# apple/ml-4m

Hardware: AMD Instinct MI355X
Metric: multimodal tokens/sec (4M-B train step, whole job) (higher is better)
Workload: dtype bf16; 1 GPU; 4M-B mod7 (fm_base_12e_12d_swiglu_nobias, 360.8M params, 8 input / 7 target modalities) masked-modeling train step, 224^2 token grids, 128 input + 128 target tokens/sample, AdamW; model=fm_base_12e_12d_swiglu_nobias, per_gpu_batch=256, global_batch=256, seq_len=256, parallelism=dp1

## Files before the change

include/fourm_hip.h:

```cpp
#ifndef FOURM_HIP_H
#define FOURM_HIP_H
#include <stdint.h>

#ifdef __cplusplus
extern "C" {
#endif

#define FM_ABI_VERSION 11
int fm_abi_version(void);
const char* fm_last_error(void);

enum fm_epilogue {
    FM_EPI_BF16 = 0,
    FM_EPI_GELU = 1,
    FM_EPI_RESIDUAL = 2,
    FM_EPI_SWIGLU = 3,
    FM_EPI_F32 = 4,
    FM_EPI_TANH = 5,
    FM_EPI_SWIGLU_BWD = 6,
    FM_EPI_GELU_BWD = 7,
    FM_EPI_QUICK_GELU = 8,
    FM_EPI_RELU = 9,
    FM_EPI_RELU_BWD = 10
};
// ... 97 lines not shown
    FM_KIND_SEQ = 2,
    FM_KIND_SEQ_EMB = 3
};
typedef struct fm_mod_desc {
    const void* ids;
    const void* mask;
    const void* dam;
    const void* table;
    const void* pos;
    const void* mod_emb;
    const void* proj_bias;
    int32_t L;
    int32_t kind, ids_are_i64, mod_id;
    int32_t max_len;
    int32_t shifted;
    int32_t mask_stride, id_stride;
    int32_t patch, channels, grid_w, orig_dim;
    int32_t head_index;
    int32_t pad_;
} fm_mod_desc;

typedef struct fm_select_desc {
    fm_mod_desc mods[FM_MAX_MODS];
    int32_t n_mods, batch, dim, n_keep, n_reg, total_len, is_decoder;
    int32_t raw;
    const void* reg_tokens;
    const void* mask_token;
    void* tokens;
    void* emb;
    void* x0;
    void* out_mask;
    void* out_mod;
    void* slot_mod;
    void* slot_src;
    void* slot_pos;
    void* target_ids;
    void* out_cs;
    void* out_mod_pre;
    void* out_mod_index;
    void* patch_rows;
    void* seqemb_rows;
    int32_t patch_ld, seqemb_ld;
    int32_t rows_f32;
    int32_t pad2_;
} fm_select_desc;
int fm_select_embed(const fm_select_desc* desc, void* stream);

typedef struct fm_embed_bwd_mod {
    void* d_table;
    void* d_pos;
    void* d_mod_emb;
    void* d_proj_bias;
    int32_t kind, has_padding_idx, padding_idx, pad_;
} fm_embed_bwd_mod;
typedef struct fm_embed_bwd_desc {
    fm_embed_bwd_mod mods[FM_MAX_MODS];
    const void* dx;
    const void* slot_mod; const void* slot_src; const void* slot_pos;
    void* d_mask_token;
    void* d_reg_tokens;
    int32_t n_mods, batch, dim, Nt, lddx, is_decoder;
} fm_embed_bwd_desc;
int fm_embed_bwd(const fm_embed_bwd_desc* desc, void* stream);

int fm_dense_decoder_mask(const int32_t* cs, const int16_t* mod, void* out, int B, int M, int causal, int use_cs,
                          int use_sep, void* stream);

enum fm_loss_type { FM_LOSS_MOD = 0, FM_LOSS_TOKEN = 1 };
#define FM_SEG_ROWS 256
int fm_segment_rows(const int32_t* head_of_row, int R, int n_heads, int32_t* seg_start, int32_t* seg_count,
                    int32_t* perm, int32_t* row_to_padded, int32_t* tile_group, int Rp, void* stream);
int fm_gather_rows(const void* src, int ld_src, const int32_t* perm, void* dst, int ld_dst, int Rp, int D, void* stream);
int fm_cross_entropy(void* logits, int ldl, const int32_t* perm, const int32_t* tile_group, const int64_t* target_ids,
                     const int32_t* vocab, const int32_t* seg_start, const int32_t* seg_count, const void* grad_scale,
                     int loss_type, int n_heads, int Rp, int max_vocab, void* row_loss, void* row_lse, void* head_loss,
                     void* total_loss, int write_grad, void* stream);

int fm_swiglu_bwd(const void* da, int ldda, const void* gu, int ldgu, void* dgu, int lddgu, int R, int H, int Hp, void* stream);
int fm_gelu_bwd(const void* dh, int lddh, const void* pre, int ldp, void* dpre, int lddp, int R, int H, int Hp, void* stream);
typedef struct fm_shadow_desc {
    const void* src; void* dst;
    int32_t ld_src, ld_dst, rows, cols, transpose, tile_start;
    const void* col_scale;
    int32_t dst_f32, reserved;
} fm_shadow_desc;
int fm_shadow_refresh(const fm_shadow_desc* descs, int n_descs, int total_tiles, void* stream);
#define FM_FOLD_MAX_JOBS 48
typedef struct fm_fold_grad_job {
    const void* dWp; const void* W; const void* gamma; void* gW; void* ggamma;
    int32_t rows, cols, ld_dwp, reserved;
} fm_fold_grad_job;
int fm_fold_colscale_grad(const fm_fold_grad_job* jobs, int n_jobs, void* stream);

int fm_cast_pad(const void* src, int ld_src, void* dst, int ld_dst, int rows, int cols, void* stream);
int fm_transpose_cast_pad(const void* src, int ld_src, void* dst, int ld_dst, int dst_cols, int rows, int cols, void* stream);
int fm_colsum(const void* dy, int ldy, void* db, int R, int N, void* stream);
int fm_f32_to_bf16(const void* src, void* dst, int64_t n, void* stream);
int fm_bf16_to_f32_scaled(const void* src, void* dst, int64_t n, float scale, void* stream);
int fm_add_bf16_f32(const void* x, const void* delta, void* out, int64_t n, void* stream);
int fm_scale_rows_bf16(void* x, int ld, const void* scale, int rows_per_sample, int R, int N, void* stream);

int fm_vit_patch_rows(const void* pixels, void* rows, int ld, int B, int C, int H, int W, int P, int rows_f32, void* stream);
int fm_vit_emb_rows(const void* pos, const void* mod_emb, void* x, int ldx, int B, int Np, int D, void* stream);
int fm_vit_colsum(const void* dy, int ldy, void* db, int R, int N, void* ws, int64_t ws_bytes, void* stream);

int fm_clip_embed_ln(const void* patches, int ldp, int patches_f32, const void* cls, const void* pos, const void* w, const void* b,
                     void* out, int ldo, int B, int G, int D, float eps, void* stream);

enum { FM_FEAT_COSINE = 0, FM_FEAT_L1 = 1 };
int fm_feat_distance(const void* pred, int ldp, const void* tgt, int ldt, int B, int T, int D, int mode, void* loss, void* dpred, int lddp,
                     void* stream);
int fm_quick_gelu_bwd(const void* da, int ldda, const void* pre, int ldp, void* dpre, int lddp, int R, int H, int Hp, void* stream);
int fm_quick_gelu_bwd_f32(const void* da, int ldda, const void* pre, int ldp, void* dpre, int lddp, int R, int H, void* stream);
int fm_clip_embed_ln_bwd(const void* dy, int lddy, const void* patches, int ldp, int patches_f32, const void* pos, const void* w,
                         void* d_patches, int lddp, int B, int G, int D, float eps, void* stream);
int fm_tap_add(void* g, int ldg, void* g_bf, int ldgb, const void* dtap, int ldt, const void* row_scale, int rows_per_sample, int R, int D,
               void* stream);

#define FM_LPIPS_CHUNK 64
int fm_lpips_stem(const void* img, const void* mul, const void* add, const void* w, const void* bias, void* out, int ldo, int is_f32, int B, int H,
                  int W, void* stream);
int fm_lpips_stem_bwd(const void* d, int ldd, int is_f32, const void* w, const void* mul, const void* row_scale, void* dimg, int B, int H, int W,
                      void* stream);
int fm_maxpool2x2_nhwc(const void* x, int ldx, void* y, int ldy, int is_f32, int B, int H, int W, int C, void* stream);
int fm_lpips_distance(const void* pred, int ldp, const void* tgt, int ldt, int is_f32, const void* w, int B, int P, int C, void* loss, void* dpred,
                      int lddp, void* scratch, void* stream);
int fm_lpips_tap_bwd(const void* act, int lda, const void* din, int ldi, const void* dtap, int ldt, const void* dpool, int ldp, void* d, int ldd,
                     int is_f32, int B, int H, int W, int C, void* stream);

int fm_lora_apply(const void* x, int ldx, const void* down, int64_t down_sr, int64_t down_sk, const void* up, int64_t up_sn, int64_t up_sr,
                  void* y, int ldy, float scale, void* p_out, int R, int K, int N, int r, int x_f32, int y_f32, void* stream);
int fm_lora_grad(const void* a, int lda, const void* b, void* out, int64_t out_sn, int64_t out_sr, float scale, int accumulate,
                 int R, int n, int r, int a_f32, void* stream);

int fm_adamw(void* p, const void* g, void* m, void* v, int64_t n, float lr, float beta1, float beta2, float eps,
             float weight_decay, int64_t step, const void* grad_mult, const void* hyper, void* sumsq, void* stream);
#define FM_ADAMW_CHUNK 8192
typedef struct fm_adamw_job {
    void* p; const void* g; void* m; void* v; void* dst_plain; void* dst_t;
    int32_t rows, cols, ld_plain, ld_t, tile_start, pad_;
} fm_adamw_job;
int fm_adamw_shadow(const fm_adamw_job* jobs, int n_jobs, int total_tiles, float lr, float beta1, float beta2, float eps,
                    float weight_decay, int64_t step, const void* grad_mult, const void* hyper, void* sumsq, void* stream);
int fm_sumsq(const void* x, int64_t n, void* out, void* stream);
int fm_clip_coef(const void* sumsq, float max_norm, void* norm_out, void* coef_out, void* stream);

int fm_sample_tokens(const void* logits, int ld, int logits_are_f32, int R, int V, float temperature, int top_k, float top_p,
                     const void* uniforms, void* out_ids, void* out_prob, void* stream);
int fm_guidance_combine(const void* uncond, int ldu, int uncond_is_f32, const void* cond, int ldc, int cond_is_f32, float weight,
                        void* out, int ldo, int R, int V, int accumulate, void* stream);
int fm_maskgit_commit(const void* prob, const void* samples, const int32_t* mod_pos, int B, int N, int num_select, void* tensor,
                      int tensor_is_i64, int L, void* input_mask, void* target_mask, int32_t* top_idx, void* stream);

typedef struct fm_gemm_f32_args {
    const void* X; const void* W; const void* W2; void* out; void* out2; const void* res; const void* bias; const void* bias2;
    int64_t sxm, sxk, swn, swk;
    int32_t M, N, K, ldo, ldo2, ldr, Hp, epilogue, accumulate, max_N, seg_rows, n_groups;
    const fm_gemm_group* groups; const int32_t* tile_group; const int32_t* seg_start; const int32_t* seg_count;
} fm_gemm_f32_args;
int fm_gemm_f32(const fm_gemm_f32_args* args, void* stream);
int fm_attn_f32_fwd(const fm_attn_args* args, void* stream);
int fm_attn_f32_bwd(const fm_attn_args* args, void* stream);
int fm_layernorm_bwd_f32(const void* dy, int lddy, const int32_t* dy_row_map, const void* x, int ldx, const void* w, const void* mean,
                         const void* rstd, const void* dres, void* dx, int lddx, void* dx2, int lddx2, void* dw, void* db, int R, int D,
                         void* stream);
int fm_headnorm_f32_fwd(const void* x, int ldx, const void* w, const void* b, void* y, int ldy, void* stats, int R, int H, float eps, void* stream);
int fm_headnorm_f32_bwd(const void* dy, int lddy, const void* x, int ldx, const void* w, const void* stats, void* dx, int lddx, void* dw, void* db,
// ... 198 lines not shown
```

ml-4m_amd/csrc/elementwise.hip:

```cpp
#include "common.h"
#include "fourm_hip.h"

namespace {

__device__ __forceinline__ float4 ld_bf4(const bf16_t* p) {
    const uint2 v = *(const uint2*)p;
    return make_float4(bf2f((bf16_t)(v.x & 0xffff)), bf2f((bf16_t)(v.x >> 16)), bf2f((bf16_t)(v.y & 0xffff)), bf2f((bf16_t)(v.y >> 16)));
}
__device__ __forceinline__ void st_bf4(bf16_t* p, float a, float b, float c, float d) {
    *(uint2*)p = make_uint2(pack2bf(a, b), pack2bf(c, d));
}
__device__ __forceinline__ float sigmoid_f(float x) { return 1.0f / (1.0f + __expf(-x)); }

__global__ __launch_bounds__(256) void swiglu_bwd_kernel(const bf16_t* __restrict__ da, int ldda, const bf16_t* __restrict__ gu, int ldgu,
                                                         bf16_t* __restrict__ dgu, int lddgu, int R, int H, int Hp, int nt) {
    const int cpr = Hp / 8;
    const size_t total = (size_t)R * cpr;
    for (size_t i = (size_t)blockIdx.x * 256 + threadIdx.x; i < total; i += (size_t)gridDim.x * 256) {
        const int r = i / cpr, c = (i % cpr) * 8;
        typedef __attribute__((ext_vector_type(4))) unsigned int u4_t;
        uint4 dp, gp, up;
        if (nt & 2) { const u4_t t = __builtin_nontemporal_load((const u4_t*)(da + (size_t)r * ldda + c)); dp = make_uint4(t[0], t[1], t[2], t[3]); }
        else dp = *(const uint4*)(da + (size_t)r * ldda + c);
        if (nt & 1) {
            const u4_t t = __builtin_nontemporal_load((const u4_t*)(gu + (size_t)r * ldgu + c)), v = __builtin_nontemporal_load((const u4_t*)(gu + (size_t)r * ldgu + Hp + c));
            gp = make_uint4(t[0], t[1], t[2], t[3]); up = make_uint4(v[0], v[1], v[2], v[3]);
        } else { gp = *(const uint4*)(gu + (size_t)r * ldgu + c); up = *(const uint4*)(gu + (size_t)r * ldgu + Hp + c); }
        const uint32_t dw[4] = {dp.x, dp.y, dp.z, dp.w}, gw[4] = {gp.x, gp.y, gp.z, gp.w}, uw[4] = {up.x, up.y, up.z, up.w};
        uint32_t og[4], ou[4];
#pragma unroll
        for (int q = 0; q < 4; ++q) {
            float dg[2], du[2];
#pragma unroll
            for (int e = 0; e < 2; ++e) {
                const float dv = bf2f((bf16_t)(e ? dw[q] >> 16 : dw[q] & 0xffff));
                const float gv = bf2f((bf16_t)(e ? gw[q] >> 16 : gw[q] & 0xffff));
                const float uv = bf2f((bf16_t)(e ? uw[q] >> 16 : uw[q] & 0xffff));
                const float sg = sigmoid_f(gv);
                const float sl = bfround(gv * sg);
                const float ds = bfround(dv * uv);
                const bool live = c + 2 * q + e < H;
                du[e] = live ? dv * sl : 0.f;
                dg[e] = live ? ds * (sg * (1.0f + gv * (1.0f - sg))) : 0.f;
            }
            og[q] = pack2bf(dg[0], dg[1]); ou[q] = pack2bf(du[0], du[1]);
        }
        *(uint4*)(dgu + (size_t)r * lddgu + c) = make_uint4(og[0], og[1], og[2], og[3]);
        *(uint4*)(dgu + (size_t)r * lddgu + Hp + c) = make_uint4(ou[0], ou[1], ou[2], ou[3]);
    }
}

__global__ __launch_bounds__(256) void gelu_bwd_kernel(const bf16_t* __restrict__ dh, int lddh, const bf16_t* __restrict__ pre, int ldp,
                                                       bf16_t* __restrict__ dpre, int lddp, int R, int H, int Hp) {
    const int cpr = Hp / 4;
    const size_t total = (size_t)R * cpr;
    for (size_t i = (size_t)blockIdx.x * 256 + threadIdx.x; i < total; i += (size_t)gridDim.x * 256) {
        const int r = i / cpr, c = (i % cpr) * 4;
        const float4 d = ld_bf4(dh + (size_t)r * lddh + c), x = ld_bf4(pre + (size_t)r * ldp + c);
        const float dv[4] = {d.x, d.y, d.z, d.w}, xv[4] = {x.x, x.y, x.z, x.w};
        float o[4];
#pragma unroll
        for (int e = 0; e < 4; ++e) {
            const float cdf = 0.5f * (1.0f + erf_fast(xv[e] * 0.70710678118654752f));
            const float pdf = 0.3989422804014327f * __expf(-0.5f * xv[e] * xv[e]);
            o[e] = (c + e < H) ? dv[e] * (cdf + xv[e] * pdf) : 0.f;
        }
        st_bf4(dpre + (size_t)r * lddp + c, o[0], o[1], o[2], o[3]);
    }
}

template <bool F32>
__global__ __launch_bounds__(256) void quick_gelu_bwd_kernel(const void* __restrict__ da_, int ldda, const void* __restrict__ pre_, int ldp,
                                                             void* __restrict__ dpre_, int lddp, int R, int H, int Hp) {
    if constexpr (F32) {
        const float *da = (const float*)da_, *pre = (const float*)pre_;
        float* dpre = (float*)dpre_;
        const size_t total = (size_t)R * H;
        for (size_t i = (size_t)blockIdx.x * 256 + threadIdx.x; i < total; i += (size_t)gridDim.x * 256) {
            const size_t r = i / H, c = i % H;
            const float u = pre[r * ldp + c];
            const float s = 1.0f / (1.0f + expf(-1.702f * u));
            dpre[r * lddp + c] = da[r * ldda + c] * (s * (1.0f + 1.702f * u * (1.0f - s)));
        }
    } else {
// ... 19 lines not shown

__global__ __launch_bounds__(256) void tap_add_kernel(float* __restrict__ g, int ldg, bf16_t* __restrict__ g_bf, int ldgb, const float* __restrict__ dtap, int ldt,
                                                      const float* __restrict__ row_scale, int rows_per_sample, int R, int D) {
#pragma clang fp contract(off)
    const int cpr = D / 4;
    const size_t total = (size_t)R * cpr;
    for (size_t i = (size_t)blockIdx.x * 256 + threadIdx.x; i < total; i += (size_t)gridDim.x * 256) {
        const size_t r = i / cpr;
        const int c = (int)(i % cpr) * 4;
        const float4 a = *(const float4*)(g + r * ldg + c), d = *(const float4*)(dtap + r * ldt + c);
        float4 o;
        if (row_scale) {
            const float s = row_scale[r / rows_per_sample];
            const float px = s * d.x, py = s * d.y, pz = s * d.z, pw = s * d.w;
            o = make_float4(a.x + px, a.y + py, a.z + pz, a.w + pw);
        } else {
            o = make_float4(a.x + d.x, a.y + d.y, a.z + d.z, a.w + d.w);
        }
        *(float4*)(g + r * ldg + c) = o;
        if (g_bf) st_bf4(g_bf + r * ldgb + c, o.x, o.y, o.z, o.w);
    }
}

__global__ __launch_bounds__(256) void cast_pad_kernel(const float* __restrict__ src, int lds_, bf16_t* __restrict__ dst, int ldd, int rows, int cols) {
    const int cpr = ldd / 4;
    const size_t total = (size_t)rows * cpr;
    for (size_t i = (size_t)blockIdx.x * 256 + threadIdx.x; i < total; i += (size_t)gridDim.x * 256) {
        const int r = i / cpr, c = (i % cpr) * 4;
        float v[4];
#pragma unroll
        for (int e = 0; e < 4; ++e) v[e] = (c + e < cols) ? src[(size_t)r * lds_ + c + e] : 0.f;
        st_bf4(dst + (size_t)r * ldd + c, v[0], v[1], v[2], v[3]);
    }
}

__global__ __launch_bounds__(256) void transpose_cast_kernel(const float* __restrict__ src, int lds_, bf16_t* __restrict__ dst, int ldd, int dst_cols, int rows, int cols) {
    __shared__ float tile[64][65];
    const int tr0 = blockIdx.y * 64, tc0 = blockIdx.x * 64;
    for (int i = threadIdx.x; i < 64 * 64; i += 256) {
        const int r = i / 64, c = i % 64;
        const int gr = tr0 + r, gc = tc0 + c;
        tile[r][c] = (gr < rows && gc < cols) ? src[(size_t)gr * lds_ + gc] : 0.f;
    }
    __syncthreads();
    for (int i = threadIdx.x; i < 64 * 64; i += 256) {
        const int c = i / 64, r = i % 64;
        const int gc = tc0 + c, gr = tr0 + r;
        if (gc < cols && gr < dst_cols) dst[(size_t)gc * ldd + gr] = f2bf(tile[r][c]);
    }
}

constexpr int SHADOW_TILES_PER_BLOCK = 8;

__global__ __launch_bounds__(256) void shadow_refresh_kernel(const fm_shadow_desc* __restrict__ descs, int n, int total_tiles) {
    __shared__ float tile[64][65];
    const int t_first = blockIdx.x * SHADOW_TILES_PER_BLOCK;
    int lo = 0, hi = n - 1;
    while (lo < hi) {
        const int mid = (lo + hi + 1) >> 1;
        if (descs[mid].tile_start <= t_first) lo = mid; else hi = mid - 1;
    }
    fm_shadow_desc d = descs[lo];
    int next_start = lo + 1 < n ? descs[lo + 1].tile_start : 0x7fffffff;
    const int q = (threadIdx.x & 15) * 4, p = threadIdx.x >> 4;
    for (int tt = t_first; tt < min(total_tiles, t_first + SHADOW_TILES_PER_BLOCK); ++tt) {
        if (tt >= next_start) {
            ++lo;
            d = descs[lo];
            next_start = lo + 1 < n ? descs[lo + 1].tile_start : 0x7fffffff;
        }
        const int t = tt - d.tile_start;
        const int tiles_c = (d.cols + 63) / 64;
        const int tr0 = (t / tiles_c) * 64, tc0 = (t % tiles_c) * 64;
        const float* src = (const float*)d.src;
        bf16_t* dst = (bf16_t*)d.dst;
        const bool vec_src = ((((uintptr_t)src) & 15) == 0) && (d.ld_src % 4 == 0);
        const bool vec_dst = ((((uintptr_t)dst) & 7) == 0) && (d.ld_dst % 4 == 0);
        float v[4][4];
#pragma unroll
        for (int i = 0; i < 4; ++i) {
            const int gr = tr0 + p + 16 * i, gc = tc0 + q;
#pragma unroll
            for (int e = 0; e < 4; ++e) v[i][e] = 0.f;
            if (gr < d.rows) {
                const float* sp = src + (size_t)gr * d.ld_src + gc;
                if (vec_src && gc + 3 < d.cols) {
                    const float4 f = *(const float4*)sp;
                    v[i][0] = f.x; v[i][1] = f.y; v[i][2] = f.z; v[i][3] = f.w;
                } else {
#pragma unroll
                    for (int e = 0; e < 4; ++e) if (gc + e < d.cols) v[i][e] = sp[e];
                }
            }
        }
        if (d.col_scale) {
            const float* cs = (const float*)d.col_scale;
#pragma unroll
            for (int e = 0; e < 4; ++e) {
                const float sc = tc0 + q + e < d.cols ? cs[tc0 + q + e] : 0.f;
#pragma unroll
                for (int i = 0; i < 4; ++i) v[i][e] *= sc;
            }
        }
        if (d.dst_f32) {
            float* df = (float*)d.dst;
            if (!d.transpose) {
#pragma unroll
                for (int i = 0; i < 4; ++i) {
                    const int gr = tr0 + p + 16 * i, gc = tc0 + q;
                    if (gr >= d.rows) continue;
#pragma unroll
                    for (int e = 0; e < 4; ++e) if (gc + e < d.cols) df[(size_t)gr * d.ld_dst + gc + e] = v[i][e];
                }
            } else {
#pragma unroll
                for (int i = 0; i < 4; ++i) {
                    const int gr = tr0 + p + 16 * i, gc = tc0 + q;
                    if (gr >= d.rows) continue;
#pragma unroll
                    for (int e = 0; e < 4; ++e) if (gc + e < d.cols) df[(size_t)(gc + e) * d.ld_dst + gr] = v[i][e];
                }
            }
            continue;
        }
        if (!d.transpose) {
#pragma unroll
            for (int i = 0; i < 4; ++i) {
                const int gr = tr0 + p + 16 * i, gc = tc0 + q;
                if (gr >= d.rows) continue;
                bf16_t* dp = dst + (size_t)gr * d.ld_dst + gc;
                if (vec_dst && gc + 3 < d.cols) *(uint2*)dp = make_uint2(pack2bf(v[i][0], v[i][1]), pack2bf(v[i][2], v[i][3]));
                else
#pragma unroll
                    for (int e = 0; e < 4; ++e) if (gc + e < d.cols) dp[e] = f2bf(v[i][e]);
            }
            continue;
        }
        __syncthreads();
#pragma unroll
        for (int i = 0; i < 4; ++i)
#pragma unroll
            for (int e = 0; e < 4; ++e) tile[p + 16 * i][q + e] = v[i][e];
        __syncthreads();
#pragma unroll
        for (int i = 0; i < 4; ++i) {
            const int c = p + 16 * i, gc = tc0 + c, gr = tr0 + q;
            if (gc >= d.cols) continue;
            bf16_t* dp = dst + (size_t)gc * d.ld_dst + gr;
            if (vec_dst && gr + 3 < d.rows) *(uint2*)dp = make_uint2(pack2bf(tile[q][c], tile[q + 1][c]), pack2bf(tile[q + 2][c], tile[q + 3][c]));
            else
#pragma unroll
                for (int e = 0; e < 4; ++e) if (gr + e < d.rows) dp[e] = f2bf(tile[q + e][c]);
        }
    }
}

__global__ __launch_bounds__(256) void colsum_kernel(const bf16_t* __restrict__ dy, int ldy, float* __restrict__ db, int R, int N, int rows_per_block) {
    __shared__ float red[8][256 + 8];
    const int cg = threadIdx.x & 31, rl = threadIdx.x >> 5;
    const int n0 = blockIdx.x * 256 + cg * 8;
    const int r0 = blockIdx.y * rows_per_block, r1 = min(R, r0 + rows_per_block);
    float s[8] = {0.f, 0.f, 0.f, 0.f, 0.f, 0.f, 0.f, 0.f};
    if (n0 < N) {
        const bool wide = n0 + 8 <= N && (ldy & 7) == 0 && (((uintptr_t)dy) & 15) == 0;
        for (int r = r0 + rl; r < r1; r += 8) {
            const bf16_t* row = dy + (size_t)r * ldy + n0;
            if (wide) {
                const uint4 v = *(const uint4*)row;
                const uint32_t w[4] = {v.x, v.y, v.z, v.w};
#pragma unroll
                for (int e = 0; e < 4; ++e) { s[2 * e] += bf2f((bf16_t)(w[e] & 0xffff)); s[2 * e + 1] += bf2f((bf16_t)(w[e] >> 16)); }
            } else {
                for (int e = 0; e < 8; ++e) if (n0 + e < N) s[e] += bf2f(row[e]);
            }
        }
    }
#pragma unroll
    for (int e = 0; e < 8; ++e) red[rl][cg * 8 + e] = s[e];
    __syncthreads();
    const int n = blockIdx.x * 256 + threadIdx.x;
    if (n < N) {
        float t = 0.f;
#pragma unroll
        for (int k = 0; k < 8; ++k) t += red[k][threadIdx.x];
        unsafeAtomicAdd(db + n, t);
    }
}

__global__ __launch_bounds__(256) void adamw_kernel(float* __restrict__ p, const float* __restrict__ g, float* __restrict__ m, float* __restrict__ v,
                                                    size_t n, float lr, float beta1, float beta2, float eps, float wd, float bc1, float bc2_sqrt,
                                                    const float* __restrict__ grad_mult, const float* __restrict__ hyper, float* __restrict__ sumsq) {
    if (hyper) { lr = hyper[0]; wd = hyper[1]; bc1 = hyper[2]; bc2_sqrt = hyper[3]; }
    const float gm = grad_mult ? grad_mult[0] : 1.0f;
    const float step = lr / bc1;
    float ss = 0.f;
    auto update = [&](float& pe, float& me, float& ve, float ge) {
        ss += ge * ge;
        ge *= gm;
        pe *= 1.0f - lr * wd;
        me = beta1 * me + (1.0f - beta1) * ge;
        ve = beta2 * ve + (1.0f - beta2) * ge * ge;
        pe -= step * me / (sqrtf(ve) / bc2_sqrt + eps);
    };
    auto quad = [&](size_t o, float4 P, float4 M, float4 V, float4 G) {
        update(P.x, M.x, V.x, G.x); update(P.y, M.y, V.y, G.y); update(P.z, M.z, V.z, G.z); update(P.w, M.w, V.w, G.w);
        *(float4*)(p + o) = P; *(float4*)(m + o) = M; *(float4*)(v + o) = V;
    };
    auto slow = [&](size_t o) {
        if (o + 4 <= n) quad(o, *(float4*)(p + o), *(float4*)(m + o), *(float4*)(v + o), *(const float4*)(g + o));
        else for (size_t j = o; j < n; ++j) update(p[j], m[j], v[j], g[j]);
    };
    const size_t stride = (size_t)gridDim.x * 256 * 4;
    for (size_t i = ((size_t)blockIdx.x * 256 + threadIdx.x) * 4; i < n; i += 2 * stride) {
        const size_t i2 = i + stride;
        if (i2 + 4 <= n) {
            const float4 P0 = *(float4*)(p + i), P1 = *(float4*)(p + i2), M0 = *(float4*)(m + i), M1 = *(float4*)(m + i2);
            const float4 V0 = *(float4*)(v + i), V1 = *(float4*)(v + i2), G0 = *(const float4*)(g + i), G1 = *(const float4*)(g + i2);
            quad(i, P0, M0, V0, G0);
            quad(i2, P1, M1, V1, G1);
        } else {
            slow(i);
            if (i2 < n) slow(i2);
        }
    }
    if (sumsq) {
        ss = wave_sum(ss);
        if ((threadIdx.x & 63) == 0) unsafeAtomicAdd(sumsq, ss);
    }
}

constexpr int ADAMW_CHUNK = 8192;

__global__ __launch_bounds__(256) void adamw_shadow_kernel(const fm_adamw_job* __restrict__ jobs, int n, int total_tiles, float lr, float beta1,
                                                           float beta2, float eps, float wd, float bc1, float bc2_sqrt,
                                                           const float* __restrict__ grad_mult, const float* __restrict__ hyper, float* __restrict__ sumsq) {
    if (hyper) { lr = hyper[0]; wd = hyper[1]; bc1 = hyper[2]; bc2_sqrt = hyper[3]; }
// ... 116 lines not shown
inline int grid_for(size_t work_items) {
    size_t g = (work_items + 255) / 256;
    if (g > 256 * 8) g = 256 * 8;
    if (g < 1) g = 1;
    return (int)g;
}

}

extern "C" int fm_swiglu_bwd(const void* da, int ldda, const void* gu, int ldgu, void* dgu, int lddgu, int R, int H, int Hp, void* stream) {
    FM_CHECK_ARG(da && gu && dgu && R > 0 && H > 0 && Hp >= H && Hp % 8 == 0, "fm_swiglu_bwd: bad argument (Hp must be a multiple of 8)");
    FM_CHECK_ARG(ldda % 8 == 0 && ldgu % 8 == 0 && lddgu % 8 == 0 && ((((uintptr_t)da | (uintptr_t)gu | (uintptr_t)dgu) & 15) == 0),
                 "fm_swiglu_bwd: 16-byte aligned buffers with leading dims that are multiples of 8");
    static const int ew_nt = [] { const char* e = getenv("FOURM_EW_NT"); return e ? atoi(e) : 3; }();
    hipLaunchKernelGGL(swiglu_bwd_kernel, dim3(grid_for((size_t)R * Hp / 8)), dim3(256), 0, (hipStream_t)stream, (const bf16_t*)da, ldda,
                       (const bf16_t*)gu, ldgu, (bf16_t*)dgu, lddgu, R, H, Hp, ew_nt);
    FM_CHECK_LAUNCH("fm_swiglu_bwd");
    return 0;
}

extern "C" int fm_gelu_bwd(const void* dh, int lddh, const void* pre, int ldp, void* dpre, int lddp, int R, int H, int Hp, void* stream) {
    FM_CHECK_ARG(dh && pre && dpre && R > 0 && H > 0 && Hp >= H && Hp % 4 == 0, "fm_gelu_bwd: bad argument");
    FM_CHECK_ARG(lddh % 4 == 0 && ldp % 4 == 0 && lddp % 4 == 0, "fm_gelu_bwd: leading dims must be multiples of 4");
    hipLaunchKernelGGL(gelu_bwd_kernel, dim3(grid_for((size_t)R * Hp / 4)), dim3(256), 0, (hipStream_t)stream, (const bf16_t*)dh, lddh,
                       (const bf16_t*)pre, ldp, (bf16_t*)dpre, lddp, R, H, Hp);
    FM_CHECK_LAUNCH("fm_gelu_bwd");
    return 0;
}

extern "C" int fm_quick_gelu_bwd(const void* da, int ldda, const void* pre, int ldp, void* dpre, int lddp, int R, int H, int Hp, void* stream) {
    FM_CHECK_ARG(da && pre && dpre, "fm_quick_gelu_bwd: null pointer");
    FM_CHECK_ARG(R > 0 && H > 0 && Hp >= H && Hp % 4 == 0, "fm_quick_gelu_bwd: R=%d H=%d Hp=%d: positive sizes, Hp >= H a multiple of 4", R, H, Hp);
    FM_CHECK_ARG(ldda % 4 == 0 && ldp % 4 == 0 && lddp % 4 == 0 && ldda >= Hp && ldp >= Hp && lddp >= Hp,
                 "fm_quick_gelu_bwd: leading dims %d %d %d must be multiples of 4 and >= Hp=%d", ldda, ldp, lddp, Hp);
    FM_CHECK_ARG(((((uintptr_t)da) | ((uintptr_t)pre) | ((uintptr_t)dpre)) & 7) == 0, "fm_quick_gelu_bwd: pointers must be 8-byte aligned");
    hipLaunchKernelGGL(quick_gelu_bwd_kernel<false>, dim3(grid_for((size_t)R * Hp / 4)), dim3(256), 0, (hipStream_t)stream, da, ldda, pre, ldp, dpre, lddp,
                       R, H, Hp);
    FM_CHECK_LAUNCH("fm_quick_gelu_bwd");
    return 0;
}

extern "C" int fm_quick_gelu_bwd_f32(const void* da, int ldda, const void* pre, int ldp, void* dpre, int lddp, int R, int H, void* stream) {
    FM_CHECK_ARG(da && pre && dpre, "fm_quick_gelu_bwd_f32: null pointer");
    FM_CHECK_ARG(R > 0 && H > 0 && ldda >= H && ldp >= H && lddp >= H, "fm_quick_gelu_bwd_f32: R=%d H=%d positive, leading dims %d %d %d >= H", R, H, ldda,
                 ldp, lddp);
    hipLaunchKernelGGL(quick_gelu_bwd_kernel<true>, dim3(grid_for((size_t)R * H)), dim3(256), 0, (hipStream_t)stream, da, ldda, pre, ldp, dpre, lddp, R, H, H);
    FM_CHECK_LAUNCH("fm_quick_gelu_bwd_f32");
    return 0;
}

extern "C" int fm_tap_add(void* g, int ldg, void* g_bf, int ldgb, const void* dtap, int ldt, const void* row_scale, int rows_per_sample, int R, int D,
                          void* stream) {
    FM_CHECK_ARG(g && dtap, "fm_tap_add: null pointer");
    FM_CHECK_ARG(R > 0 && D > 0 && D % 4 == 0, "fm_tap_add: R=%d D=%d: positive, D a multiple of 4", R, D);
    FM_CHECK_ARG(!row_scale || rows_per_sample > 0, "fm_tap_add: rows_per_sample=%d must be positive with row_scale", rows_per_sample);
    FM_CHECK_ARG(ldg >= D && ldt >= D && ldg % 4 == 0 && ldt % 4 == 0 && (!g_bf || (ldgb >= D && ldgb % 4 == 0)),
                 "fm_tap_add: leading dims %d %d %d must be multiples of 4 and >= D=%d", ldg, ldt, ldgb, D);
    FM_CHECK_ARG(((((uintptr_t)g) | ((uintptr_t)dtap)) & 15) == 0 && (((uintptr_t)g_bf) & 7) == 0 && (((uintptr_t)row_scale) & 3) == 0,
                 "fm_tap_add: g / dtap must be 16-byte aligned, g_bf 8-byte aligned");
    hipLaunchKernelGGL(tap_add_kernel, dim3(grid_for((size_t)R * D / 4)), dim3(256), 0, (hipStream_t)stream, (float*)g, ldg, (bf16_t*)g_bf, ldgb,
                       (const float*)dtap, ldt, (const float*)row_scale, row_scale ? rows_per_sample : 1, R, D);
    FM_CHECK_LAUNCH("fm_tap_add");
    return 0;
}

extern "C" int fm_cast_pad(const void* src, int ld_src, void* dst, int ld_dst, int rows, int cols, void* stream) {
    FM_CHECK_ARG(src && dst && rows > 0 && cols > 0 && ld_dst >= cols && ld_dst % 4 == 0, "fm_cast_pad: bad argument");
    hipLaunchKernelGGL(cast_pad_kernel, dim3(grid_for((size_t)rows * ld_dst / 4)), dim3(256), 0, (hipStream_t)stream, (const float*)src, ld_src,
                       (bf16_t*)dst, ld_dst, rows, cols);
    FM_CHECK_LAUNCH("fm_cast_pad");
    return 0;
}

extern "C" int fm_transpose_cast_pad(const void* src, int ld_src, void* dst, int ld_dst, int dst_cols, int rows, int cols, void* stream) {
    FM_CHECK_ARG(src && dst && rows > 0 && cols > 0 && dst_cols >= rows && ld_dst >= dst_cols, "fm_transpose_cast_pad: bad argument");
    dim3 grid((cols + 63) / 64, (dst_cols + 63) / 64);
    hipLaunchKernelGGL(transpose_cast_kernel, grid, dim3(256), 0, (hipStream_t)stream, (const float*)src, ld_src, (bf16_t*)dst, ld_dst, dst_cols, rows, cols);
    FM_CHECK_LAUNCH("fm_transpose_cast_pad");
    return 0;
}

extern "C" int fm_shadow_refresh(const fm_shadow_desc* descs, int n_descs, int total_tiles, void* stream) {
    FM_CHECK_ARG(descs && n_descs > 0 && total_tiles > 0, "fm_shadow_refresh: bad argument");
    hipLaunchKernelGGL(shadow_refresh_kernel, dim3((total_tiles + SHADOW_TILES_PER_BLOCK - 1) / SHADOW_TILES_PER_BLOCK), dim3(256), 0,
                       (hipStream_t)stream, descs, n_descs, total_tiles);
    FM_CHECK_LAUNCH("fm_shadow_refresh");
    return 0;
}

struct FoldArgs { fm_fold_grad_job job[FM_FOLD_MAX_JOBS]; int n; };
__global__ __launch_bounds__(256) void fold_colscale_grad_kernel(FoldArgs a) {
    __shared__ float red[4][64];
    const fm_fold_grad_job j = a.job[blockIdx.z];
    const int cl = threadIdx.x & 63, rl = threadIdx.x >> 6;
    const int c = blockIdx.x * 64 + cl, r0 = blockIdx.y * 64;
    float s = 0.f;
    if (c < j.cols && r0 < j.rows) {
        const float g = ((const float*)j.gamma)[c];
        const float* dwp = (const float*)j.dWp;
        const float* w = (const float*)j.W;
        float* gw = (float*)j.gW;
        const int r1 = min(j.rows, r0 + 64);
        for (int r = r0 + rl; r < r1; r += 4) {
            const float d = dwp[(size_t)r * j.ld_dwp + c];
            if (gw) gw[(size_t)r * j.cols + c] += d * g;
            s += d * w[(size_t)r * j.cols + c];
        }
    }
    red[rl][cl] = s;
    __syncthreads();
    if (rl == 0 && c < j.cols && j.ggamma && r0 < j.rows) atomicAdd((float*)j.ggamma + c, red[0][cl] + red[1][cl] + red[2][cl] + red[3][cl]);
}

extern "C" int fm_fold_colscale_grad(const fm_fold_grad_job* jobs, int n_jobs, void* stream) {
    FM_CHECK_ARG(jobs && n_jobs > 0 && n_jobs <= FM_FOLD_MAX_JOBS, "fm_fold_colscale_grad: 1..FM_FOLD_MAX_JOBS jobs");
    FoldArgs a{};
    int max_r = 0, max_c = 0;
    for (int i = 0; i < n_jobs; ++i) {
        const fm_fold_grad_job& j = jobs[i];
        FM_CHECK_ARG(j.dWp && j.W && j.gamma && j.rows > 0 && j.cols > 0 && j.ld_dwp >= j.cols, "fm_fold_colscale_grad: bad job");
        a.job[i] = j;
        max_r = j.rows > max_r ? j.rows : max_r;
        max_c = j.cols > max_c ? j.cols : max_c;
    }
    a.n = n_jobs;
    hipLaunchKernelGGL(fold_colscale_grad_kernel, dim3((max_c + 63) / 64, (max_r + 63) / 64, n_jobs), dim3(256), 0, (hipStream_t)stream, a);
    FM_CHECK_LAUNCH("fm_fold_colscale_grad");
    return 0;
}

extern "C" int fm_colsum(const void* dy, int ldy, void* db, int R, int N, void* stream) {
    FM_CHECK_ARG(dy && db && R > 0 && N > 0, "fm_colsum: bad argument");
    const int rpb = 128;
    dim3 grid((N + 255) / 256, (R + rpb - 1) / rpb);
    hipLaunchKernelGGL(colsum_kernel, grid, dim3(256), 0, (hipStream_t)stream, (const bf16_t*)dy, ldy, (float*)db, R, N, rpb);
    FM_CHECK_LAUNCH("fm_colsum");
    return 0;
}

extern "C" int fm_adamw(void* p, const void* g, void* m, void* v, int64_t n, float lr, float beta1, float beta2, float eps,
                        float weight_decay, int64_t step, const void* grad_mult, const void* hyper, void* sumsq, void* stream) {
    FM_CHECK_ARG(p && g && m && v && n > 0 && step > 0, "fm_adamw: bad argument");
    FM_CHECK_ARG((((uintptr_t)p | (uintptr_t)g | (uintptr_t)m | (uintptr_t)v) & 15) == 0, "fm_adamw: buffers must be 16-byte aligned");
    const double bc1 = 1.0 - pow((double)beta1, (double)step), bc2 = 1.0 - pow((double)beta2, (double)step);
    hipLaunchKernelGGL(adamw_kernel, dim3(grid_for((size_t)(n + 3) / 4)), dim3(256), 0, (hipStream_t)stream, (float*)p, (const float*)g, (float*)m,
                       (float*)v, (size_t)n, lr, beta1, beta2, eps, weight_decay, (float)bc1, (float)sqrt(bc2), (const float*)grad_mult,
                       (const float*)hyper, (float*)sumsq);
    FM_CHECK_LAUNCH("fm_adamw");
    return 0;
}

extern "C" int fm_adamw_shadow(const fm_adamw_job* jobs, int n_jobs, int total_tiles, float lr, float beta1, float beta2, float eps,
                               float weight_decay, int64_t step, const void* grad_mult, const void* hyper, void* sumsq, void* stream) {
    FM_CHECK_ARG(jobs && n_jobs > 0 && total_tiles > 0 && step > 0, "fm_adamw_shadow: bad argument");
    const double bc1 = 1.0 - pow((double)beta1, (double)step), bc2 = 1.0 - pow((double)beta2, (double)step);
    const int blocks = total_tiles < 8192 ? total_tiles : 8192;
    hipLaunchKernelGGL(adamw_shadow_kernel, dim3(blocks), dim3(256), 0, (hipStream_t)stream, jobs, n_jobs, total_tiles, lr, beta1, beta2, eps,
                       weight_decay, (float)bc1, (float)sqrt(bc2), (const float*)grad_mult, (const float*)hyper, (float*)sumsq);
    FM_CHECK_LAUNCH("fm_adamw_shadow");
    return 0;
}

extern "C" int fm_sumsq(const void* x, int64_t n, void* out, void* stream) {
    FM_CHECK_ARG(x && out && n > 0 && (((uintptr_t)x) & 15) == 0, "fm_sumsq: bad argument");
    hipLaunchKernelGGL(sumsq_kernel, dim3(grid_for((size_t)(n + 3) / 4)), dim3(256), 0, (hipStream_t)stream, (const float*)x, (size_t)n, (float*)out);
    FM_CHECK_LAUNCH("fm_sumsq");
    return 0;
}
// ... 60 lines not shown
```

ml-4m_amd/csrc/gemm.hip:

```cpp
#include <type_traits>
#include <cstdlib>
#include <algorithm>
#include "common.h"
#include "fourm_hip.h"
#include "gemm_args.h"

namespace {
using namespace fmk;

constexpr int BK = 64;

__device__ __attribute__((aligned(16))) const uint32_t g_zero16[4] = {0u, 0u, 0u, 0u};

template <int TW, int TX, int WW, int WX, int KB, int STAGES, int EPI, bool GROUPED, bool PP = false, bool PERSIST = false, bool CONV = false>
__global__ __launch_bounds__(WW * WX * 64) void gemm_nt_kernel(NTArgs a) {
    constexpr int NWAVES = WW * WX;
    constexpr int RB = KB * 2;
    constexpr int CPR = RB / 16;
    constexpr int RPP = 1024 / RB;
    constexpr int SWSH = (RB == 128) ? 1 : 2;
    constexpr int LOADS = (TW + TX) / (RPP * NWAVES);
    constexpr int FW = TW / WW / 32, FX = TX / WX / 32;
    constexpr int STAGE = (TW + TX) * RB;
    static_assert(TW % (RPP * NWAVES) == 0 && TX % (RPP * NWAVES) == 0, "tile rows must split evenly over the DMA pieces");
// ... 897 lines not shown
        for (int i = 0; i < FWA; ++i)
#pragma unroll
            for (int jj = 0; jj < 2; ++jj)
#pragma unroll
                for (int r = 0; r < 16; ++r) acc[i][jj][r] = 0.f;

        const int NT_ = t_end - t_begin;
#pragma unroll
        for (int p = 0; p < STAGES - 1; ++p)
            if (p < NT_) stage(t_begin + p, p);
        if (NT_ > 1) wait_vmcnt<LOADS>(); else wait_vmcnt<0>();
        block_barrier();
        if (!lead) block_barrier();
        int buf = 0;
        for (int it = 0; it < NT_; ++it) {
            const bool more = it + 2 < NT_;
            const int nbuf = buf >= 1 ? buf - 1 : 2;
            const uint32_t st = smem_lds + buf * STAGE;
            union Frag { bf16x8_t v; s16x4_t h[2]; };
            Frag af[KS][FWA], bfr[KS][2];
            auto read_k = [&](auto kk_c) {
                constexpr int kk = decltype(kk_c)::value;
#pragma unroll
                for (int i = 0; i < FWA; ++i) {
                    af[kk][i].h[0] = tr_read<kk * 16 * RBA>(st + baseA[i]);
                    af[kk][i].h[1] = tr_read<kk * 16 * RBA + 4 * RBA>(st + baseA[i]);
                }
#pragma unroll
                for (int jj = 0; jj < 2; ++jj) {
                    bfr[kk][jj].h[0] = tr_read<kk * 16 * RBB>(st + baseB[jj]);
                    bfr[kk][jj].h[1] = tr_read<kk * 16 * RBB + 4 * RBB>(st + baseB[jj]);
                }
            };
            read_k(std::integral_constant<int, 0>{});
            read_k(std::integral_constant<int, 1>{});
            if constexpr (KS > 2) read_k(std::integral_constant<int, 2>{});
            if constexpr (KS > 3) read_k(std::integral_constant<int, 3>{});
            if (!lead) {
                if (more) { stage(t_begin + it + 2, nbuf); wait_vmcnt<LOADS>(); } else wait_vmcnt<0>();
            }
            wait_lgkmcnt<0>();
            block_barrier();
            __builtin_amdgcn_sched_barrier(0);
            __builtin_amdgcn_s_setprio(1);
#pragma unroll
            for (int kk = 0; kk < KS; ++kk) {
#pragma unroll
                for (int i = 0; i < FWA; ++i)
#pragma unroll
                    for (int jj = 0; jj < 2; ++jj)
                        acc[i][jj] = __builtin_amdgcn_mfma_f32_32x32x16_bf16(af[kk][i].v, bfr[kk][jj].v, acc[i][jj], 0, 0, 0);
                if (lead && more) stage_part(t_begin + it + 2, nbuf, kk, KS);
            }
            __builtin_amdgcn_s_setprio(0);
            if (lead) { if (more) wait_vmcnt<LOADS>(); else wait_vmcnt<0>(); }
            __builtin_amdgcn_sched_barrier(0);
            if (lead || it + 1 < NT_) block_barrier();
            buf = buf + 1 == STAGES ? 0 : buf + 1;
        }
        float* out = jb.out;
        const int N = jb.N, K = jb.K, ldo = jb.ldo;
        if (a.lab & 1) return;
#pragma unroll
        for (int jj = 0; jj < 2; ++jj) {
            const int k = k0 + wb * 64 + jj * 32 + (lane & 31);
            if (k >= K) continue;
#pragma unroll
            for (int i = 0; i < FWA; ++i)
#pragma unroll
                for (int r = 0; r < 16; ++r) {
                    const int n = n0 + wa * (TA / 2) + i * 32 + (r & 3) + 8 * (r >> 2) + 4 * fhi;
                    if (n < N) unsafeAtomicAdd(out + (size_t)n * ldo + k, acc[i][jj][r]);
                }
        }
    };
    tn_multi_walk(a, w, G, run);
}

int g_nt_config = 9, g_nt_prio = 1;
int g_lab[16] = {0, 0, [] { const char* e = getenv("FOURM_NT3"); return e ? atoi(e) : 3; }(), [] { const char* e = getenv("FOURM_NT3_LAB"); return e ? atoi(e) : 0; }(),
                 [] { const char* e = getenv("FOURM_NT4"); return e ? atoi(e) : 1; }(),
                 [] { const char* e = getenv("FOURM_TN4"); return e ? atoi(e) : 0; }(), 0, 0, 0,
                 [] { const char* e = getenv("FOURM_NT_SMALL"); return e ? atoi(e) : 1; }(),
                 [] { const char* e = getenv("FOURM_CONV_K32"); return e ? atoi(e) : 1; }()};
int g_nt_swiglu = 12;
int g_nt_auto[2] = {11, 10};

int g_reserved_cus = [] { const char* e = getenv("FOURM_RESERVED_CUS"); return e ? atoi(e) : 0; }();
static int n_compute_units() {
    static int n = [] {
        int dev = 0, cus = 0;
        if (hipGetDevice(&dev) != hipSuccess || hipDeviceGetAttribute(&cus, hipDeviceAttributeMultiprocessorCount, dev) != hipSuccess || cus <= 0) cus = 256;
        return cus;
    }();
    const int avail = n - g_reserved_cus;
    return avail >= 64 ? avail / 8 * 8 : n;
}

}
int fm_grid_cus() { return n_compute_units(); }
namespace {

template <int TW, int TX, int WW, int WX, int KB, int STAGES, int EPI, bool GROUPED, bool PP = false, bool PERSIST = false, bool CONV = false>
int launch_nt_cfg(NTArgs a, int max_n, hipStream_t s) {
    constexpr int NPT = (EPI == EPI_SWIGLU) ? TW / 2 : TW;
    a.n_tiles_w = (max_n + NPT - 1) / NPT;
    a.n_tiles_x = (a.M + TX - 1) / TX;
    int grid = a.n_tiles_w * a.n_tiles_x;
    if (GROUPED) {
        const int gw_max = TW > 128 ? 8 : 16;
        a.group_w = a.n_tiles_w < gw_max ? a.n_tiles_w : gw_max;
        const int chunks = ((a.n_tiles_w + a.group_w - 1) / a.group_w) * ((a.n_tiles_x + 3) / 4);
        grid = (chunks + 7) / 8 * 8 * a.group_w * 4;
    }
    const size_t lds = (size_t)STAGES * (TW + TX) * KB * 2;
    if (PERSIST) {
        const int slots = n_compute_units() * (int)(160 * 1024 / lds) / 8 * 8;
        if (grid > slots) grid = slots;
    }
    auto k = gemm_nt_kernel<TW, TX, WW, WX, KB, STAGES, EPI, GROUPED, PP, PERSIST, CONV>;
    static bool once = (hipFuncSetAttribute((const void*)k, hipFuncAttributeMaxDynamicSharedMemorySize, (int)lds), true);
    (void)once;
    hipLaunchKernelGGL(k, dim3(grid, a.split_k > 1 ? a.split_k : 1), dim3(WW * WX * 64), lds, s, a);
    FM_CHECK_LAUNCH("fm_gemm_nt");
    return 0;
}

__global__ __launch_bounds__(256) void splitk_reduce_kernel(const float* __restrict__ ws, int S, long long stride, int M, int N4, int ldp, const float* __restrict__ bias,
                                                            bf16_t* __restrict__ out, int ldo) {
    const long long total = (long long)M * N4;
    for (long long e = (long long)blockIdx.x * 256 + threadIdx.x; e < total; e += (long long)gridDim.x * 256) {
        const int m = (int)(e / N4), n = (int)(e % N4) * 4;
        float4 acc = *(const float4*)(ws + (size_t)m * ldp + n);
        for (int z = 1; z < S; ++z) {
            const float4 t = *(const float4*)(ws + (size_t)z * stride + (size_t)m * ldp + n);
            acc.x += t.x; acc.y += t.y; acc.z += t.z; acc.w += t.w;
        }
        if (bias) { const float4 b = *(const float4*)(bias + n); acc.x += bfround(b.x); acc.y += bfround(b.y); acc.z += bfround(b.z); acc.w += bfround(b.w); }
        *(uint2*)(out + (size_t)m * ldo + n) = make_uint2(pack2bf(acc.x, acc.y), pack2bf(acc.z, acc.w));
    }
}

template <int EPI, bool GROUPED>
int launch_nt(const NTArgs& a, int max_n, hipStream_t s) {
    if constexpr (GROUPED) {
        static_assert(FM_SEG_ROWS == 256, "the grouped configurations use a 256-row X tile");
        if constexpr (EPI == EPI_BF16) {
            static const int heads_cfg_k = [] { const char* e = getenv("FOURM_HEADS_NT_CFG"); return e ? atoi(e) : 0; }();
            if (a.K >= 1536 && heads_cfg_k == 3) return launch_nt_cfg<256, 256, 2, 4, 32, 3, EPI, true, true>(a, max_n, s);
            if (a.K >= 1536 && heads_cfg_k == 4) return launch_nt_cfg<256, 256, 2, 4, 64, 2, EPI, true>(a, max_n, s);
        }
        if (a.K >= 1536) return launch_nt_cfg<128, 256, 2, 4, 64, 3, EPI, true, true>(a, max_n, s);
        if constexpr (EPI == EPI_BF16) {
            static const int heads_cfg = [] { const char* e = getenv("FOURM_HEADS_NT_CFG"); return e ? atoi(e) : 0; }();
            if (heads_cfg == 1) return launch_nt_cfg<256, 256, 2, 4, 32, 3, EPI, true, true>(a, max_n, s);
            if (heads_cfg == 2) return launch_nt_cfg<128, 256, 2, 4, 32, 3, EPI, true, true>(a, max_n, s);
        }
        return launch_nt_cfg<128, 256, 2, 4, 32, 3, EPI, true>(a, max_n, s);
    }
    if (a.M <= 128 || a.fixed_tiling) return launch_nt_cfg<128, 128, 2, 2, 32, 3, EPI, GROUPED>(a, max_n, s);
    if constexpr (!GROUPED) {
        int cfg = g_nt_config;
        if (cfg == 9) {
            cfg = EPI == EPI_SWIGLU ? g_nt_swiglu : g_nt_auto[(a.K >= 1536 || EPI == EPI_RES || EPI == EPI_SWIGLU_BWD || EPI == EPI_GELU_BWD) ? 1 : 0];
            const long t256 = (long)((max_n + 255) / 256) * ((a.M + 255) / 256);
            if (cfg == g_nt_auto[0] && g_nt_auto[0] == 11 && max_n % 256 == 0 && t256 % n_compute_units() == 0) cfg = 12;
        }
// ... 107 lines not shown
    if (!grouped && !fixed && g_lab[9] && p->epilogue == FM_EPI_BF16 && p->M > 32 && !p->out2 && !p->res && p->N % 4 == 0 && (((uintptr_t)p->out) & 7) == 0) {
        const int cus = n_compute_units();
        const long t256 = (long)((p->M + 255) / 256) * ((p->N + 255) / 256);
        if (t256 * 2 <= cus) {
            const long t128 = (long)((p->M + 127) / 128) * ((p->N + 127) / 128);
            const int kt = p->K / 64;
            int S = 1;
            const long ldp = (p->N + 3) / 4 * 4;
            if (p->splitk_ws && t128 * 2 <= cus && kt >= 8 && p->K % 64 == 0 && (((uintptr_t)p->splitk_ws) & 15) == 0) {
                S = (int)std::min<long>({cus / t128, (long)kt / 4, 16L, (long)(p->splitk_ws_bytes / ((long long)p->M * ldp * 4))});
            }
            if (S >= 2) {
                const int ks = (kt + S - 1) / S * 64;
                S = (p->K + ks - 1) / ks;
                NTArgs b = a;
                b.out = p->splitk_ws; b.ldo = (int)ldp; b.bias = nullptr;
                b.split_k = S; b.k_slice = ks; b.split_stride = (long long)p->M * ldp;
                const int r = launch_nt_cfg<128, 128, 2, 2, 64, 3, EPI_F32, false>(b, max_n, s);
                if (r != 0) return r;
                const long long quads = (long long)p->M * (ldp / 4);
                const int rgrid = (int)std::min<long long>((quads + 255) / 256, 2048);
                hipLaunchKernelGGL(splitk_reduce_kernel, dim3(rgrid), dim3(256), 0, s, (const float*)p->splitk_ws, S, b.split_stride, p->M, (int)(ldp / 4), (int)ldp,
                                   (const float*)p->bias, (bf16_t*)p->out, p->ldo);
                FM_CHECK_LAUNCH("fm_gemm_nt (split-K reduction)");
                return 0;
            }
            if (p->K >= 1536) return launch_nt_cfg<128, 128, 2, 2, 64, 3, EPI_BF16, false>(a, max_n, s);
            return launch_nt_cfg<128, 128, 2, 2, 32, 3, EPI_BF16, false>(a, max_n, s);
        }
    }
    if (!grouped && !fixed && g_lab[4]) {
        const int r = fm_launch_nt4(a, p->epilogue, g_lab[4], s);
        if (r < 0) { fm_set_error("fm_gemm_nt (nt4): launch failed"); return -2; }
        if (r > 0) return 0;
    }
    if (!grouped && !fixed && g_lab[2]) {
        const int r = fm_launch_nt3(a, p->epilogue, g_lab[2], s);
        if (r < 0) { fm_set_error("fm_gemm_nt (nt3): launch failed"); return -2; }
        if (r > 0) return 0;
    }
    if (!grouped && !fixed && g_nt_config == 9) {
        const int r = fm_launch_nt_flat(a, p->epilogue, s);
        if (r < 0) { fm_set_error("fm_gemm_nt (flat): launch failed"); return -2; }
        if (r > 0) return 0;
    }
    if (grouped) {
        FM_CHECK_ARG(p->tile_group && p->max_N > 0, "fm_gemm_nt: grouped mode needs tile_group and max_N");
        FM_CHECK_ARG(p->epilogue == FM_EPI_BF16, "fm_gemm_nt: grouped mode supports FM_EPI_BF16 only");
        return launch_nt<EPI_BF16, true>(a, max_n, s);
    }
    switch (p->epilogue) {
        case FM_EPI_BF16: return launch_nt<EPI_BF16, false>(a, max_n, s);
        case FM_EPI_GELU: return launch_nt<EPI_GELU, false>(a, max_n, s);
        case FM_EPI_QUICK_GELU: return launch_nt<EPI_QGELU, false>(a, max_n, s);
        case FM_EPI_RESIDUAL:
            FM_CHECK_ARG(p->res && p->ldr % 4 == 0, "fm_gemm_nt: residual epilogue needs res / ldr%%4==0");
            return launch_nt<EPI_RES, false>(a, max_n, s);
        case FM_EPI_SWIGLU:
            FM_CHECK_ARG(p->W2 && p->Hp % 4 == 0 && (!p->out2 || p->ldo2 % 4 == 0), "fm_gemm_nt: SwiGLU epilogue needs W2, Hp%%4==0");
            return launch_nt<EPI_SWIGLU, false>(a, max_n, s);
        case FM_EPI_F32: return launch_nt<EPI_F32, false>(a, max_n, s);
        case FM_EPI_TANH: return launch_nt<EPI_TANH, false>(a, max_n, s);
        case FM_EPI_SWIGLU_BWD:
            FM_CHECK_ARG(p->res && p->ldr % 4 == 0 && p->Hp % 4 == 0 && p->Hp >= p->N && p->ldo >= 2 * p->Hp && p->ldr >= 2 * p->Hp,
                         "fm_gemm_nt: SwiGLU-backward epilogue needs res=(g|u) and out=(dg|du) of width 2*Hp");
            return launch_nt<EPI_SWIGLU_BWD, false>(a, max_n, s);
        case FM_EPI_GELU_BWD:
            FM_CHECK_ARG(p->res && p->ldr % 4 == 0, "fm_gemm_nt: GELU-backward epilogue needs res = pre-activation");
            return launch_nt<EPI_GELU_BWD, false>(a, max_n, s);
    }
    fm_set_error("fm_gemm_nt: unknown epilogue %d", p->epilogue);
    return -1;
}

extern int g_nt_flat;
extern "C" void fm_set_gemm_nt_config(int cfg) {
    g_nt_config = cfg & 0xff; g_nt_prio = (cfg >> 8) & 1;
    g_nt_flat = (cfg >> 29) & 1;
    if ((cfg >> 16) & 0xff) { g_nt_auto[0] = (cfg >> 16) & 0xf; g_nt_auto[1] = (cfg >> 20) & 0xf; }
    if ((cfg >> 24) & 0xf) g_nt_swiglu = (cfg >> 24) & 0xf;
}
extern "C" int fm_get_gemm_nt_config(void) { return g_nt_config; }
extern "C" void fm_lab_set(int key, int value) { if (key >= 0 && key < 16) g_lab[key] = value; }
extern "C" void fm_set_reserved_cus(int n) { g_reserved_cus = n < 0 ? 0 : n; }
extern "C" int fm_get_reserved_cus(void) { return g_reserved_cus; }
static int g_tn_config = [] { const char* e = getenv("FOURM_TN_CONFIG"); return e ? atoi(e) : 1; }();
extern "C" void fm_set_gemm_tn_config(int cfg) { g_tn_config = cfg; }
extern "C" int fm_get_gemm_tn_config(void) { return g_tn_config; }
static int g_tn_use_tr = 1;
extern "C" void fm_set_tn_transpose_read(int on) { g_tn_use_tr = on; }
extern "C" int fm_get_tn_transpose_read(void) { return g_tn_use_tr; }

extern "C" int fm_gemm_tn(const fm_gemm_tn_args* p, void* stream) {
    FM_CHECK_ARG(p && p->A && p->B, "fm_gemm_tn: null pointer");
    const bool grouped = p->groups != nullptr;
    FM_CHECK_ARG(grouped || p->out, "fm_gemm_tn: out is null");
    FM_CHECK_ARG(p->K > 0 && (grouped || (p->N > 0 && p->R > 0)), "fm_gemm_tn: bad shape");
    FM_CHECK_ARG(p->lda % 8 == 0 && p->ldb % 8 == 0, "fm_gemm_tn: leading dims must be multiples of 8");
    TNArgs a{};
    a.A = (const bf16_t*)p->A; a.B = (const bf16_t*)p->B; a.out = (float*)p->out;
    a.R = p->R; a.N = p->N; a.K = p->K; a.lda = p->lda; a.ldb = p->ldb; a.ldo = p->ldo;
    a.a_cols = p->a_cols > 0 ? p->a_cols : p->lda; a.b_cols = p->b_cols > 0 ? p->b_cols : p->ldb;
    FM_CHECK_ARG(a.a_cols >= 8 && a.b_cols >= 8, "fm_gemm_tn: operands need at least 8 readable columns");
    a.groups = p->groups; a.seg_start = p->seg_start; a.seg_count = p->seg_count;
    const int max_n = grouped ? p->max_N : p->N;
    constexpr int TN_TA = 128, TN_TB = 256, TN_STAGES = 3;
    const bool pp = (g_tn_config == 1 || g_tn_config == 3 || g_tn_config == 4) && !grouped && p->force_tr != 0;
    const int kb = pp ? 64 : 32, slots = (pp ? 1 : 2) * n_compute_units();
    a.n_tiles_a = (max_n + TN_TA - 1) / TN_TA; a.n_tiles_b = (p->K + TN_TB - 1) / TN_TB;
    int splits = p->splits;
    if (splits <= 0) {
        const int tiles = a.n_tiles_a * a.n_tiles_b;
        const int nt = grouped ? (p->max_R + kb - 1) / kb : (p->R + kb - 1) / kb;
        splits = tiles >= slots ? 1 : slots / tiles;
        while (splits > 1 && nt / splits < 8) --splits;
        if (splits > 64) splits = 64;
        if (nt < 16) splits = 1;
    }
    a.splits = splits;
    const size_t lds = (size_t)TN_STAGES * kb * (TN_TA + TN_TB) * 2;
    const int total_items = a.n_tiles_a * a.n_tiles_b * splits;
    const int deal = grouped ? 8 * 4 * a.n_tiles_b : 8;
    dim3 grid((total_items + deal - 1) / deal * deal, 1, grouped ? p->n_groups : 1);
    hipStream_t s = (hipStream_t)stream;
    const bool masked = grouped || p->R % kb != 0;
#define LAUNCH_TN(TR, G, KBV, PPV)                                                                  \
    if (masked) LAUNCH_TN2(TR, G, KBV, PPV, true) else LAUNCH_TN2(TR, G, KBV, PPV, false)
#define LAUNCH_TN2(TR, G, KBV, PPV, MK)                                                             \
    {                                                                                               \
        auto k = gemm_tn_kernel<TR, G, TN_TA, TN_TB, 2, 4, KBV, TN_STAGES, PPV, MK>;                \
        static bool once = (hipFuncSetAttribute((const void*)k, hipFuncAttributeMaxDynamicSharedMemorySize, (int)lds), true); \
        (void)once;                                                                                 \
        hipLaunchKernelGGL(k, grid, dim3(512), lds, s, a);                                          \
    }
    const int tr = p->force_tr >= 0 ? p->force_tr : g_tn_use_tr;
    if (pp) { if (grouped) { LAUNCH_TN(true, true, 64, true); } else { LAUNCH_TN(true, false, 64, true); } }
    else if (tr) { if (grouped) { LAUNCH_TN(true, true, 32, false); } else { LAUNCH_TN(true, false, 32, false); } }
    else { if (grouped) { LAUNCH_TN(false, true, 32, false); } else { LAUNCH_TN(false, false, 32, false); } }
#undef LAUNCH_TN
#undef LAUNCH_TN2
    FM_CHECK_LAUNCH("fm_gemm_tn");
    return 0;
}

extern "C" int fm_gemm_tn_multi(const fm_gemm_tn_job* jobs, int n_jobs, void* stream) {
    FM_CHECK_ARG(jobs && n_jobs > 0 && n_jobs <= FM_TN_MAX_JOBS, "fm_gemm_tn_multi: 1..FM_TN_MAX_JOBS jobs");
    TNMultiArgs a{};
    bool masked = false;
    int tiles = 0;
    long long units = 0;
    static const bool small_env = [] { const char* e = getenv("FOURM_TN_MULTI_TILE"); return e && atoi(e) == 128; }();
    const bool big = !(small_env || g_tn_config == 3);
    bool t4 = big && g_lab[5] != 0 && (g_tn_config == 1 || g_tn_config == 4);
    if (t4) {
        double useful = 0, padded = 0;
        for (int i = 0; i < n_jobs && t4; ++i) {
            const fm_gemm_tn_job& p = jobs[i];
            const int ac = p.a_cols > 0 ? p.a_cols : p.lda, bc = p.b_cols > 0 ? p.b_cols : p.ldb;
            t4 = p.R % 64 == 0 && p.R >= 256 && p.N % 128 == 0 && p.K % 128 == 0 && ac >= 128 && bc >= 128 && ac % 8 == 0 && bc % 8 == 0 &&
                 (((uintptr_t)p.A | (uintptr_t)p.B) & 15) == 0 && ((size_t)p.R * p.lda + ac) * 2 < 0x7fffffffull && ((size_t)p.R * p.ldb + bc) * 2 < 0x7fffffffull;
            useful += (double)p.N * p.K * p.R;
            padded += (double)((p.N + 255) / 256 * 256) * ((p.K + 383) / 384 * 384) * p.R;
        }
        t4 = t4 && useful >= 0.92 * padded;
    }
    const bool ls = big && (g_tn_config == 4 || t4);
// ... 80 lines not shown
```

ml-4m_amd/csrc/loss.hip:

```cpp
#include "common.h"
#include "fourm_hip.h"

namespace {

constexpr int SEG_ALIGN = FM_SEG_ROWS;

__global__ __launch_bounds__(1024) void segment_rows_kernel(const int32_t* __restrict__ head_of_row, int R, int n_heads,
                                                            int32_t* __restrict__ seg_start, int32_t* __restrict__ seg_count,
                                                            int32_t* __restrict__ perm, int32_t* __restrict__ row_to_padded,
                                                            int32_t* __restrict__ tile_group, int Rp) {
    __shared__ int cnt[FM_MAX_MODS];
    __shared__ int wtot[16];
    const int g = blockIdx.x, tid = threadIdx.x, lane = tid & 63, wave = tid >> 6;
    if (tid < FM_MAX_MODS) cnt[tid] = 0;
    __syncthreads();
    for (int r = tid; r < R; r += 1024) {
        const int hh = head_of_row[r];
        if (hh >= 0 && hh <= g) atomicAdd(&cnt[hh], 1);
    }
    __syncthreads();
    int start = 0;
    for (int m = 0; m < g; ++m) start += (cnt[m] + SEG_ALIGN - 1) / SEG_ALIGN * SEG_ALIGN;
    const int mine = cnt[g];
    const int padded = (mine + SEG_ALIGN - 1) / SEG_ALIGN * SEG_ALIGN;
    if (tid == 0) { seg_start[g] = start; seg_count[g] = mine; }
    for (int t = tid; t < padded / SEG_ALIGN; t += 1024) tile_group[start / SEG_ALIGN + t] = g;
    if (g == n_heads - 1) {
        for (int t = (start + padded) / SEG_ALIGN + tid; t < Rp / SEG_ALIGN; t += 1024) tile_group[t] = -1;
        for (int r = start + padded + tid; r < Rp; r += 1024) perm[r] = -1;
    }
    for (int r = start + mine + tid; r < start + padded; r += 1024) perm[r] = -1;
    int run = 0;
    for (int base = 0; base < R; base += 1024) {
        const int r = base + tid;
        const int f = (r < R && head_of_row[r] == g) ? 1 : 0;
        const int inc = wave_scan_incl(f);
        if (lane == 63) wtot[wave] = inc;
        __syncthreads();
        int off = 0, tot = 0;
        for (int w = 0; w < 16; ++w) { if (w < wave) off += wtot[w]; tot += wtot[w]; }
        __syncthreads();
        if (f) {
            const int dst = start + run + off + inc - 1;
            perm[dst] = r;
            row_to_padded[r] = dst;
        }
        run += tot;
    }
}

__global__ void fill_i32_kernel(int32_t* p, int v, int n) {
    const int i = blockIdx.x * 256 + threadIdx.x;
    if (i < n) p[i] = v;
}

__device__ __forceinline__ void online_merge(float& m, float& s, float m2, float s2) {
    const float mn = fmaxf(m, m2);
    s = s * __expf(m - mn) + s2 * __expf(m2 - mn);
    m = mn;
}

__global__ __launch_bounds__(256) void ce_fwd_kernel(const bf16_t* __restrict__ logits, int ldl, const int32_t* __restrict__ perm,
                                                     const int32_t* __restrict__ tile_group, const long long* __restrict__ target_ids,
                                                     const int32_t* __restrict__ vocab, float* __restrict__ row_loss, float* __restrict__ row_lse) {
    __shared__ float red_m[4], red_s[4];
    const int pr = blockIdx.x;
    const int g = tile_group[pr / SEG_ALIGN];
    if (g < 0) return;
    const int src = perm[pr];
    if (src < 0) {
        if (threadIdx.x == 0) { row_loss[pr] = 0.f; row_lse[pr] = 0.f; }
        return;
    }
    const int V = vocab[g];
    const bf16_t* row = logits + (size_t)pr * ldl;
    float m = -INFINITY, ssum = 0.f;
    for (int c = threadIdx.x * 8; c < V; c += 256 * 8) {
        float v[8];
        if (c + 8 <= V) {
            const uint4 p = *(const uint4*)(row + c);
            const uint32_t w[4] = {p.x, p.y, p.z, p.w};
#pragma unroll
            for (int e = 0; e < 4; ++e) { v[2 * e] = bf2f((bf16_t)(w[e] & 0xffff)); v[2 * e + 1] = bf2f((bf16_t)(w[e] >> 16)); }
        } else {
#pragma unroll
            for (int e = 0; e < 8; ++e) v[e] = c + e < V ? bf2f(row[c + e]) : -INFINITY;
        }
        float cm = v[0];
#pragma unroll
        for (int e = 1; e < 8; ++e) cm = fmaxf(cm, v[e]);
        const float mn = fmaxf(m, cm);
        float add = 0.f;
#pragma unroll
        for (int e = 0; e < 8; ++e) add += __expf(v[e] - mn);
        ssum = ssum * __expf(m - mn) + add;
        m = mn;
    }
#pragma unroll
    for (int o = 32; o > 0; o >>= 1) {
        const float m2 = __shfl_xor(m, o, 64), s2 = __shfl_xor(ssum, o, 64);
        if (m2 > -INFINITY || m > -INFINITY) online_merge(m, ssum, m2, s2);
    }
    const int lane = threadIdx.x & 63, wave = threadIdx.x >> 6;
    if (lane == 0) { red_m[wave] = m; red_s[wave] = ssum; }
    __syncthreads();
    if (threadIdx.x == 0) {
        float M = red_m[0], S = red_s[0];
        for (int w = 1; w < 4; ++w)
            if (red_m[w] > -INFINITY) online_merge(M, S, red_m[w], red_s[w]);
        const float lse = M + __logf(S);
        row_lse[pr] = lse;
        row_loss[pr] = lse - bf2f(row[target_ids[src]]);
    }
}

__global__ __launch_bounds__(256) void ce_bwd_kernel(bf16_t* __restrict__ logits, int ldl, const int32_t* __restrict__ perm,
                                                     const int32_t* __restrict__ tile_group, const long long* __restrict__ target_ids,
                                                     const int32_t* __restrict__ vocab, const int32_t* __restrict__ seg_count,
                                                     const float* __restrict__ gscale, int loss_type, int n_heads,
                                                     const float* __restrict__ row_lse) {
    const int pr = blockIdx.x;
    const int g = tile_group[pr / SEG_ALIGN];
    if (g < 0) return;
    const int V = vocab[g];
    const int Vp = (V + 63) / 64 * 64;
    bf16_t* row = logits + (size_t)pr * ldl;
    const int src = perm[pr];
    if (src < 0) {
        for (int c = threadIdx.x; c < Vp / 8; c += 256) *(uint4*)(row + c * 8) = make_uint4(0u, 0u, 0u, 0u);
        return;
    }
    float w;
    if (loss_type == FM_LOSS_MOD) {
        w = 1.0f / ((float)seg_count[g] * (float)n_heads);
    } else {
        float tot = 0.f;
        for (int mm = 0; mm < n_heads; ++mm) tot += (float)seg_count[mm] * (float)vocab[mm];
        w = (float)V / tot;
    }
    w *= gscale ? gscale[0] : 1.0f;
    const float lse = row_lse[pr];
    const int tgt = (int)target_ids[src];
    for (int c = threadIdx.x * 8; c < Vp; c += 256 * 8) {
        const uint4 p = *(const uint4*)(row + c);
        const uint32_t wd[4] = {p.x, p.y, p.z, p.w};
        float o[8];
#pragma unroll
        for (int e = 0; e < 8; ++e) {
            const float x = bf2f((bf16_t)((e & 1) ? (wd[e >> 1] >> 16) : (wd[e >> 1] & 0xffff)));
            o[e] = (c + e < V) ? (__expf(x - lse) - ((c + e) == tgt ? 1.f : 0.f)) * w : 0.f;
        }
        *(uint4*)(row + c) = make_uint4(pack2bf(o[0], o[1]), pack2bf(o[2], o[3]), pack2bf(o[4], o[5]), pack2bf(o[6], o[7]));
    }
}

__global__ __launch_bounds__(256) void loss_finalize_kernel(const float* __restrict__ row_loss, const int32_t* __restrict__ seg_start,
                                                            const int32_t* __restrict__ seg_count, const int32_t* __restrict__ vocab,
                                                            int n_heads, int loss_type, float* __restrict__ head_loss, float* __restrict__ total) {
    __shared__ float red[4];
    __shared__ float hl[FM_MAX_MODS];
    const int lane = threadIdx.x & 63, wave = threadIdx.x >> 6;
    for (int g = 0; g < n_heads; ++g) {
        const int s0 = seg_start[g], n = seg_count[g];
        float s = 0.f;
        for (int i = threadIdx.x; i < n; i += 256) s += row_loss[s0 + i];
        s = wave_sum(s);
        if (lane == 0) red[wave] = s;
        __syncthreads();
        if (threadIdx.x == 0) hl[g] = n > 0 ? ((red[0] + red[1]) + (red[2] + red[3])) / (float)n : 0.f;
        __syncthreads();
    }
    if (threadIdx.x == 0) {
        float tot = 0.f, wsum = 0.f;
        for (int g = 0; g < n_heads; ++g) {
            head_loss[g] = hl[g];
            if (loss_type == FM_LOSS_MOD) { tot += hl[g]; wsum += 1.f; }
            else { const float w = (float)seg_count[g] * (float)vocab[g]; tot += hl[g] * w; wsum += w; }
        }
        total[0] = tot / wsum;
    }
}

__global__ __launch_bounds__(256) void ce_f32_kernel(float* logits, int ld, const int* perm, const int* tile_group, const long long* target_ids,
                                                     const int* vocab, const int* seg_count, const float* grad_scale, int loss_type, int n_heads,
                                                     float* row_loss, float* row_lse, int write_grad, int seg_rows) {
    __shared__ float red[4];
    const int pr = blockIdx.x;
    const int g = tile_group[pr / seg_rows];
    if (g < 0) return;
    const int src = perm[pr];
    const int V = vocab[g];
    float* row = logits + (size_t)pr * ld;
    if (src < 0) {
        if (!write_grad) { if (threadIdx.x == 0) { row_loss[pr] = 0.f; row_lse[pr] = 0.f; } }
        else for (int c = threadIdx.x; c < V; c += 256) row[c] = 0.f;
        return;
    }
    const int tgt = (int)target_ids[src];
    if (!write_grad) {
        float mx = -INFINITY;
        for (int c = threadIdx.x; c < V; c += 256) mx = fmaxf(mx, row[c]);
        mx = wave_max(mx);
        __syncthreads();
        if ((threadIdx.x & 63) == 0) red[threadIdx.x >> 6] = mx;
        __syncthreads();
        mx = fmaxf(fmaxf(red[0], red[1]), fmaxf(red[2], red[3]));
        float s = 0.f;
        for (int c = threadIdx.x; c < V; c += 256) s += expf(row[c] - mx);
        s = wave_sum(s);
        __syncthreads();
        if ((threadIdx.x & 63) == 0) red[threadIdx.x >> 6] = s;
        __syncthreads();
        s = (red[0] + red[1]) + (red[2] + red[3]);
        const float lse = mx + logf(s);
        if (threadIdx.x == 0) { row_lse[pr] = lse; row_loss[pr] = lse - row[tgt]; }
        return;
    }
    float coef;
    if (loss_type == FM_LOSS_MOD) coef = 1.0f / ((float)n_heads * (float)seg_count[g]);
    else {
        double tot = 0.0;
        for (int h = 0; h < n_heads; ++h) tot += (double)seg_count[h] * (double)vocab[h];
        coef = (float)((double)V / tot);
    }
    coef *= grad_scale ? grad_scale[0] : 1.0f;
    const float lse = row_lse[pr];
    for (int c = threadIdx.x; c < V; c += 256) row[c] = coef * (expf(row[c] - lse) - (c == tgt ? 1.0f : 0.f));
}


__global__ __launch_bounds__(256) void gather_rows_kernel(const bf16_t* __restrict__ src, int lds_, const int32_t* __restrict__ perm,
                                                          bf16_t* __restrict__ dst, int ldd, int Rp, int D) {
    const int lane = threadIdx.x & 63, wave = threadIdx.x >> 6;
    for (int pr = blockIdx.x * 4 + wave; pr < Rp; pr += gridDim.x * 4) {
        const int s = perm[pr];
        for (int c = lane; c < D / 8; c += 64) {
            uint4 v = make_uint4(0u, 0u, 0u, 0u);
            if (s >= 0) v = *(const uint4*)(src + (size_t)s * lds_ + c * 8);
            *(uint4*)(dst + (size_t)pr * ldd + c * 8) = v;
        }
    }
}

}

extern "C" int fm_segment_rows(const int32_t* head_of_row, int R, int n_heads, int32_t* seg_start, int32_t* seg_count,
                               int32_t* perm, int32_t* row_to_padded, int32_t* tile_group, int Rp, void* stream) {
    FM_CHECK_ARG(head_of_row && seg_start && seg_count && perm && row_to_padded && tile_group, "fm_segment_rows: null pointer");
    FM_CHECK_ARG(n_heads > 0 && n_heads <= FM_MAX_MODS && R > 0, "fm_segment_rows: bad shape");
    FM_CHECK_ARG(Rp % SEG_ALIGN == 0 && Rp >= (R + SEG_ALIGN - 1) / SEG_ALIGN * SEG_ALIGN + (n_heads - 1) * SEG_ALIGN,
                 "fm_segment_rows: padded capacity Rp=%d too small for R=%d rows in %d segments", Rp, R, n_heads);
    hipLaunchKernelGGL(fill_i32_kernel, dim3((R + 255) / 256), dim3(256), 0, (hipStream_t)stream, row_to_padded, -1, R);
    hipLaunchKernelGGL(segment_rows_kernel, dim3(n_heads), dim3(1024), 0, (hipStream_t)stream, head_of_row, R, n_heads, seg_start,
                       seg_count, perm, row_to_padded, tile_group, Rp);
    FM_CHECK_LAUNCH("fm_segment_rows");
    return 0;
}

extern "C" int fm_gather_rows(const void* src, int ld_src, const int32_t* perm, void* dst, int ld_dst, int Rp, int D, void* stream) {
    FM_CHECK_ARG(src && perm && dst && D % 8 == 0 && ld_src % 8 == 0 && ld_dst % 8 == 0, "fm_gather_rows: bad argument");
    int grid = (Rp + 3) / 4;
    if (grid > 4096) grid = 4096;
    hipLaunchKernelGGL(gather_rows_kernel, dim3(grid), dim3(256), 0, (hipStream_t)stream, (const bf16_t*)src, ld_src, perm, (bf16_t*)dst, ld_dst, Rp, D);
    FM_CHECK_LAUNCH("fm_gather_rows");
    return 0;
}

extern "C" int fm_cross_entropy(void* logits, int ldl, const int32_t* perm, const int32_t* tile_group, const int64_t* target_ids,
                                const int32_t* vocab, const int32_t* seg_start, const int32_t* seg_count, const void* grad_scale,
                                int loss_type, int n_heads, int Rp, int max_vocab, void* row_loss, void* row_lse, void* head_loss,
                                void* total_loss, int write_grad, void* stream) {
    FM_CHECK_ARG(logits && perm && tile_group && target_ids && vocab && seg_start && seg_count && row_loss && row_lse && head_loss && total_loss,
                 "fm_cross_entropy: null pointer");
    FM_CHECK_ARG(loss_type == FM_LOSS_MOD || loss_type == FM_LOSS_TOKEN, "fm_cross_entropy: invalid loss type %d", loss_type);
    FM_CHECK_ARG(ldl % 8 == 0 && ldl >= (max_vocab + 63) / 64 * 64, "fm_cross_entropy: ldl=%d too small for vocab %d", ldl, max_vocab);
    FM_CHECK_ARG((((uintptr_t)logits) & 15) == 0, "fm_cross_entropy: logits must be 16-byte aligned");
    if (!write_grad) {
        hipLaunchKernelGGL(ce_fwd_kernel, dim3(Rp), dim3(256), 0, (hipStream_t)stream, (const bf16_t*)logits, ldl, perm, tile_group,
                           (const long long*)target_ids, vocab, (float*)row_loss, (float*)row_lse);
        hipLaunchKernelGGL(loss_finalize_kernel, dim3(1), dim3(256), 0, (hipStream_t)stream, (const float*)row_loss, seg_start, seg_count,
                           vocab, n_heads, loss_type, (float*)head_loss, (float*)total_loss);
    } else {
        hipLaunchKernelGGL(ce_bwd_kernel, dim3(Rp), dim3(256), 0, (hipStream_t)stream, (bf16_t*)logits, ldl, perm, tile_group,
                           (const long long*)target_ids, vocab, seg_count, (const float*)grad_scale, loss_type, n_heads, (const float*)row_lse);
    }
    FM_CHECK_LAUNCH("fm_cross_entropy");
    return 0;
}

extern "C" int fm_cross_entropy_f32(void* logits, int ldl, const int32_t* perm, const int32_t* tile_group, const int64_t* target_ids,
                                    const int32_t* vocab, const int32_t* seg_start, const int32_t* seg_count, const void* grad_scale,
                                    int loss_type, int n_heads, int Rp, int max_vocab, void* row_loss, void* row_lse, void* head_loss,
                                    void* total_loss, int write_grad, void* stream) {
    FM_CHECK_ARG(logits && perm && tile_group && target_ids && vocab && seg_start && seg_count && row_loss && row_lse && head_loss && total_loss,
                 "fm_cross_entropy_f32: null pointer");
    FM_CHECK_ARG(loss_type == FM_LOSS_MOD || loss_type == FM_LOSS_TOKEN, "fm_cross_entropy_f32: invalid loss type %d", loss_type);
    FM_CHECK_ARG(ldl >= max_vocab, "fm_cross_entropy_f32: ldl=%d too small for vocab %d", ldl, max_vocab);
    hipLaunchKernelGGL(ce_f32_kernel, dim3(Rp), dim3(256), 0, (hipStream_t)stream, (float*)logits, ldl, perm, tile_group,
                       (const long long*)target_ids, vocab, seg_count, (const float*)grad_scale, loss_type, n_heads, (float*)row_loss,
                       (float*)row_lse, write_grad, SEG_ALIGN);
    if (!write_grad)
        hipLaunchKernelGGL(loss_finalize_kernel, dim3(1), dim3(256), 0, (hipStream_t)stream, (const float*)row_loss, seg_start, seg_count,
                           vocab, n_heads, loss_type, (float*)head_loss, (float*)total_loss);
    FM_CHECK_LAUNCH("fm_cross_entropy_f32");
    return 0;
}
```

ml-4m_amd/csrc/select_embed.hip:

```cpp
#include "common.h"
#include "fourm_hip.h"

namespace {

constexpr int MAXPOS = 8192;
constexpr int MAXKEEP = 1024;

struct SelArgs {
    fm_select_desc d;
};

__device__ __forceinline__ long long load_id(const void* ids, int is64, size_t i) {
    return is64 ? ((const long long*)ids)[i] : (long long)((const int*)ids)[i];
}

__device__ __forceinline__ int block_scan_excl(int v, int* wave_tot , int* total) {
    const int lane = threadIdx.x & 63, wave = threadIdx.x >> 6;
    const int inc = wave_scan_incl(v);
    if (lane == 63) wave_tot[wave] = inc;
    __syncthreads();
    int base = 0, tot = 0;
#pragma unroll
    for (int w = 0; w < 4; ++w) {
        const int t = wave_tot[w];
        if (w < wave) base += t;
        tot += t;
    }
    __syncthreads();
    *total = tot;
    return base + inc - v;
}

__global__ __launch_bounds__(256) void select_embed_kernel(SelArgs A) {
    const fm_select_desc& d = A.d;
    extern __shared__ __attribute__((aligned(16))) char smem[];
    const int P = d.total_len;
    int* rank_sel = (int*)smem;
    int* rank_pos = rank_sel + P;
    int* slot_p = rank_pos + P;
    uint8_t* flag = (uint8_t*)(slot_p + d.n_keep);
    __shared__ int wave_tot[4];
    __shared__ int mod_off[FM_MAX_MODS + 1];
    __shared__ int cs_scan[MAXKEEP];

    const int b = blockIdx.x;
    const int tid = threadIdx.x, lane = tid & 63, wave = tid >> 6;
    if (tid == 0) {
        int o = 0;
        for (int m = 0; m < d.n_mods; ++m) { mod_off[m] = o; o += d.mods[m].L; }
        mod_off[d.n_mods] = o;
    }
    __syncthreads();

    auto mod_of = [&](int p) {
        int m = 0;
        while (m + 1 < d.n_mods && p >= mod_off[m + 1]) ++m;
        return m;
    };

    int run_sel = 0, run_pos = 0;
    for (int base = 0; base < P; base += 256) {
        const int p = base + tid;
        int sel = 0, um = 0;
        if (p < P) {
            const int m = mod_of(p);
            const fm_mod_desc& md = d.mods[m];
            const int j = p - mod_off[m];
            const uint8_t* mk = (const uint8_t*)md.mask + (size_t)b * md.mask_stride;
            if (d.is_decoder && md.shifted) {
                um = mk[j] == 0;
                sel = (mk[j] == 0) && (mk[j + 1] == 0);
            } else {
                um = sel = mk[j] == 0;
            }
            flag[p] = (uint8_t)(sel | (um << 1));
        }
        int ts, tp;
        const int es = block_scan_excl(sel, wave_tot, &ts);
        const int ep = block_scan_excl(um, wave_tot, &tp);
        if (p < P) { rank_sel[p] = run_sel + es; rank_pos[p] = run_pos + ep; }
        run_sel += ts; run_pos += tp;
    }
    const int n_valid = run_sel;
    __syncthreads();
// ... 163 lines not shown
__global__ __launch_bounds__(256) void embed_bwd_kernel(fm_embed_bwd_desc d) {
    extern __shared__ __attribute__((aligned(16))) char smem[];
    float* acc = (float*)smem;
    const int D = d.dim, nch = D >> 2;
    const int b = blockIdx.x, lane = threadIdx.x & 63, wave = threadIdx.x >> 6;
    const int rows = d.n_mods + 1;
    for (int i = threadIdx.x; i < rows * D; i += 256) acc[i] = 0.f;
    __shared__ int used[FM_MAX_MODS + 1];
    if (threadIdx.x <= FM_MAX_MODS) used[threadIdx.x] = 0;
    __syncthreads();
    constexpr int MAXQ = 8;
    const int parts = 4 * gridDim.y, part = wave + 4 * blockIdx.y;
    const int per = (d.Nt + parts - 1) / parts, s_lo = part * per, s_hi = min(d.Nt, s_lo + per);
    float4 racc[MAXQ];
    int cur = -1;
    bool cur_mask = false;
    auto flush = [&]() {
        if (cur < 0) return;
#pragma unroll
        for (int q = 0; q < MAXQ; ++q) {
            const int c = lane + 64 * q;
            if (c >= nch) break;
            float* a0 = acc + (size_t)cur * D + c * 4;
            atomicAdd(a0, racc[q].x); atomicAdd(a0 + 1, racc[q].y); atomicAdd(a0 + 2, racc[q].z); atomicAdd(a0 + 3, racc[q].w);
            if (cur_mask) {
                float* a1 = acc + (size_t)d.n_mods * D + c * 4;
                atomicAdd(a1, racc[q].x); atomicAdd(a1 + 1, racc[q].y); atomicAdd(a1 + 2, racc[q].z); atomicAdd(a1 + 3, racc[q].w);
            }
        }
    };
    for (int s = s_lo; s < s_hi; ++s) {
        const size_t row = (size_t)b * d.Nt + s;
        const int m = ((const int32_t*)d.slot_mod)[row];
        if (m == -1) continue;
        const float* g = (const float*)d.dx + row * d.lddx;
        if (m == -2) {
            if (d.d_reg_tokens)
                for (int c = lane; c < D; c += 64) unsafeAtomicAdd((float*)d.d_reg_tokens + (size_t)s * D + c, g[c]);
            continue;
        }
        const fm_embed_bwd_mod& md = d.mods[m];
        const int src = ((const int32_t*)d.slot_src)[row];
        const int posrow = ((const int32_t*)d.slot_pos)[row];
        const bool to_mask_token = d.is_decoder && md.kind == FM_KIND_TOK;
        if (m != cur) {
            flush();
            cur = m; cur_mask = to_mask_token;
#pragma unroll
            for (int q = 0; q < MAXQ; ++q) racc[q] = make_float4(0.f, 0.f, 0.f, 0.f);
            if (lane == 0) { used[m] = 1; if (to_mask_token) used[d.n_mods] = 1; }
        }
        float* trow = nullptr;
        if (to_mask_token) {}
        else if ((md.kind == FM_KIND_TOK || md.kind == FM_KIND_SEQ) && md.d_table && !(md.has_padding_idx && src == md.padding_idx))
            trow = (float*)md.d_table + (size_t)src * D;
        else if (md.kind == FM_KIND_SEQ_EMB && md.d_proj_bias) trow = (float*)md.d_proj_bias;
        float* prow = md.d_pos ? (float*)md.d_pos + (size_t)posrow * D : nullptr;
#pragma unroll
        for (int q = 0; q < MAXQ; ++q) {
            const int c = lane + 64 * q;
            if (c >= nch) break;
            const float4 v = *(const float4*)(g + c * 4);
            racc[q].x += v.x; racc[q].y += v.y; racc[q].z += v.z; racc[q].w += v.w;
            if (trow) {
                unsafeAtomicAdd(trow + c * 4, v.x); unsafeAtomicAdd(trow + c * 4 + 1, v.y);
                unsafeAtomicAdd(trow + c * 4 + 2, v.z); unsafeAtomicAdd(trow + c * 4 + 3, v.w);
            }
            if (prow) {
                unsafeAtomicAdd(prow + c * 4, v.x); unsafeAtomicAdd(prow + c * 4 + 1, v.y);
                unsafeAtomicAdd(prow + c * 4 + 2, v.z); unsafeAtomicAdd(prow + c * 4 + 3, v.w);
            }
        }
    }
    flush();
    __syncthreads();
    for (int m = 0; m < d.n_mods; ++m) {
        if (!used[m] || !d.mods[m].d_mod_emb) continue;
        for (int c = threadIdx.x; c < D; c += 256) unsafeAtomicAdd((float*)d.mods[m].d_mod_emb + c, acc[(size_t)m * D + c]);
    }
    if (used[d.n_mods] && d.d_mask_token)
        for (int c = threadIdx.x; c < D; c += 256) unsafeAtomicAdd((float*)d.d_mask_token + c, acc[(size_t)d.n_mods * D + c]);
}

__global__ void dense_decoder_mask_kernel(const int32_t* cs, const int16_t* mod, uint8_t* out, int B, int M, int causal, int use_cs, int use_sep) {
    const size_t i = (size_t)blockIdx.x * 256 + threadIdx.x;
    if (i >= (size_t)B * M * M) return;
    const int k = i % M, q = (i / M) % M, b = i / ((size_t)M * M);
    bool blk = false;
    if (causal) blk = k > q;
    else if (use_cs) blk = k >= cs[(size_t)b * M + q];
    if (use_sep) blk = blk || (mod[(size_t)b * M + q] != mod[(size_t)b * M + k]);
    out[i] = blk ? 1 : 0;
}

}

extern "C" int fm_select_embed(const fm_select_desc* d, void* stream) {
    FM_CHECK_ARG(d && d->tokens && d->emb && d->out_mask && d->out_mod && d->slot_mod && d->slot_src && d->slot_pos, "fm_select_embed: null output");
    FM_CHECK_ARG(d->n_mods > 0 && d->n_mods <= FM_MAX_MODS, "fm_select_embed: n_mods=%d out of range (max %d)", d->n_mods, FM_MAX_MODS);
    FM_CHECK_ARG(d->dim > 0 && d->dim % 4 == 0, "fm_select_embed: dim must be a multiple of 4");
    FM_CHECK_ARG(d->batch > 0 && d->n_keep > 0 && d->n_keep <= (d->raw ? MAXPOS : MAXKEEP), "fm_select_embed: n_keep=%d out of range (max %d)", d->n_keep,
                 d->raw ? MAXPOS : MAXKEEP);
    int total = 0;
    for (int m = 0; m < d->n_mods; ++m) {
        const fm_mod_desc& md = d->mods[m];
        FM_CHECK_ARG(md.L > 0 && md.mask && md.pos && md.mod_emb, "fm_select_embed: modality %d incomplete", m);
        FM_CHECK_ARG(md.kind != FM_KIND_PATCH || (d->patch_rows && md.ids), "fm_select_embed: pixel modality needs patch_rows and pixels");
        FM_CHECK_ARG(md.kind != FM_KIND_SEQ_EMB || (d->seqemb_rows && md.ids), "fm_select_embed: seq_emb modality needs seqemb_rows");
        FM_CHECK_ARG(!((md.kind == FM_KIND_TOK || md.kind == FM_KIND_SEQ) && !(d->is_decoder && md.kind == FM_KIND_TOK)) || md.table, "fm_select_embed: modality %d needs a table", m);
        FM_CHECK_ARG(!d->is_decoder || md.dam || d->raw, "fm_select_embed: decoder modality %d needs decoder_attention_mask", m);
        FM_CHECK_ARG(!(d->raw == 2 && md.kind == FM_KIND_TOK) || md.table, "fm_select_embed: modality %d needs a table", m);
        total += md.L;
    }
    FM_CHECK_ARG(total == d->total_len, "fm_select_embed: total_len=%d but the modalities sum to %d", d->total_len, total);
    FM_CHECK_ARG(total <= MAXPOS, "fm_select_embed: %d concatenated positions exceed %d", total, MAXPOS);
    FM_CHECK_ARG(d->n_keep <= total, "fm_select_embed: n_keep=%d exceeds the %d available positions", d->n_keep, total);
    FM_CHECK_ARG(d->raw >= 0 && d->raw <= 2 && (!d->raw || (d->n_keep == total && d->n_reg == 0)),
                 "fm_select_embed: raw views cover every position (n_keep == total_len) and carry no register tokens");
    FM_CHECK_ARG(!d->is_decoder || (d->target_ids && d->out_cs && d->out_mod_pre && d->out_mod_index && d->mask_token), "fm_select_embed: decoder outputs missing");
    FM_CHECK_ARG(d->n_reg == 0 || d->reg_tokens, "fm_select_embed: register tokens missing");
    FM_CHECK_ARG(d->patch_ld % 4 == 0 && d->seqemb_ld % 4 == 0, "fm_select_embed: side buffers need ld %% 4 == 0");
    const size_t lds = (size_t)total * 9 + (size_t)d->n_keep * 4 + 16;
    static bool once = (hipFuncSetAttribute((const void*)select_embed_kernel, hipFuncAttributeMaxDynamicSharedMemorySize, MAXPOS * 9 + MAXPOS * 4 + 16) == hipSuccess);
    (void)once;
    SelArgs A; A.d = *d;
    const int slices = d->batch >= 2048 ? 1 : d->batch >= 1024 ? 2 : 4;
    hipLaunchKernelGGL(select_embed_kernel, dim3(d->batch, slices), dim3(256), lds, (hipStream_t)stream, A);
    FM_CHECK_LAUNCH("fm_select_embed");
    return 0;
}

extern "C" int fm_embed_bwd(const fm_embed_bwd_desc* d, void* stream) {
    FM_CHECK_ARG(d && d->dx && d->slot_mod && d->slot_src && d->slot_pos, "fm_embed_bwd: null pointer");
    FM_CHECK_ARG(d->n_mods > 0 && d->n_mods <= FM_MAX_MODS && d->dim % 4 == 0 && d->dim <= 2048 && d->lddx % 4 == 0, "fm_embed_bwd: bad shape (dim <= 2048)");
    const size_t lds = (size_t)(d->n_mods + 1) * d->dim * sizeof(float);
    FM_CHECK_ARG(lds <= 150 * 1024, "fm_embed_bwd: %zu bytes of LDS needed", lds);
    static bool once = (hipFuncSetAttribute((const void*)embed_bwd_kernel, hipFuncAttributeMaxDynamicSharedMemorySize, 150 * 1024) == hipSuccess);
    (void)once;
    const int slices = d->batch >= 2048 ? 1 : d->batch >= 1024 ? 2 : 4;
    hipLaunchKernelGGL(embed_bwd_kernel, dim3(d->batch, slices), dim3(256), lds, (hipStream_t)stream, *d);
    FM_CHECK_LAUNCH("fm_embed_bwd");
    return 0;
}

extern "C" int fm_dense_decoder_mask(const int32_t* cs, const int16_t* mod, void* out, int B, int M, int causal, int use_cs, int use_sep, void* stream) {
    FM_CHECK_ARG(out && (causal || !use_cs || cs) && (!use_sep || mod), "fm_dense_decoder_mask: null pointer");
    const size_t n = (size_t)B * M * M;
    hipLaunchKernelGGL(dense_decoder_mask_kernel, dim3((n + 255) / 256), dim3(256), 0, (hipStream_t)stream, cs, mod, (uint8_t*)out, B, M, causal, use_cs, use_sep);
    FM_CHECK_LAUNCH("fm_dense_decoder_mask");
    return 0;
}
```

ml-4m_amd/fourm/hip/_lib.py:

```python
import ctypes as C
import os

FM_MAX_MODS = 24
_LIB_PATH = os.environ.get("FOURM_HIP_LIB") or os.path.join(os.path.dirname(os.path.dirname(os.path.abspath(__file__))), "_lib", "libfourm_hip.so")


class FourmHipUnavailable(ImportError):
    pass


def _load():
    if not os.path.exists(_LIB_PATH):
        raise FourmHipUnavailable(
            f"{_LIB_PATH} is missing - build the gfx950 kernels first: python ml-4m_amd/build_ext.py "
            "(the 4M hot path has no fallback implementation)")
    return C.CDLL(_LIB_PATH)


lib = _load()
lib.fm_last_error.restype = C.c_char_p
lib.fm_abi_version.restype = C.c_int
ABI_VERSION = 11
if lib.fm_abi_version() != ABI_VERSION:
    raise FourmHipUnavailable(f"libfourm_hip.so ABI {lib.fm_abi_version()} != expected {ABI_VERSION}; rebuild")

vp, i32, i64, f32 = C.c_void_p, C.c_int32, C.c_int64, C.c_float

EPI_BF16, EPI_GELU, EPI_RESIDUAL, EPI_SWIGLU, EPI_F32, EPI_TANH, EPI_SWIGLU_BWD, EPI_GELU_BWD, EPI_QUICK_GELU = 0, 1, 2, 3, 4, 5, 6, 7, 8
EPI_RELU, EPI_RELU_BWD = 9, 10
MASK_NONE, MASK_KEYPAD, MASK_DECODER, MASK_DENSE = 0, 1, 2, 3
KIND_TOK, KIND_PATCH, KIND_SEQ, KIND_SEQ_EMB = 0, 1, 2, 3
LOSS_MOD, LOSS_TOKEN = 0, 1


class GemmGroup(C.Structure):
    _fields_ = [("W", vp), ("out", vp), ("N", i32), ("K", i32), ("ldw", i32), ("pad_", i32)]


class GemmNTArgs(C.Structure):
    _fields_ = [("W", vp), ("W2", vp), ("X", vp), ("out", vp), ("out2", vp), ("res", vp), ("bias", vp), ("bias2", vp),
                ("M", i32), ("N", i32), ("K", i32), ("ldw", i32), ("ldx", i32), ("ldo", i32), ("ldo2", i32), ("ldr", i32),
                ("Hp", i32), ("epilogue", i32), ("groups", vp), ("tile_group", vp), ("max_N", i32), ("fixed_tiling", i32),
                ("m_dev", vp), ("row0_dev", vp), ("splitk_ws", vp), ("splitk_ws_bytes", i64),
                ("conv_C", i32), ("conv_H", i32), ("conv_W", i32), ("conv_Ho", i32), ("conv_Wo", i32), ("conv_stride", i32), ("conv_up", i32), ("conv_pad_", i32)]


class GemmTNArgs(C.Structure):
    _fields_ = [("A", vp), ("B", vp), ("out", vp), ("R", i32), ("N", i32), ("K", i32), ("lda", i32), ("ldb", i32),
                ("ldo", i32), ("a_cols", i32), ("b_cols", i32), ("splits", i32), ("force_tr", i32), ("groups", vp),
                ("seg_start", vp), ("seg_count", vp), ("n_groups", i32), ("max_N", i32), ("max_R", i32), ("pad_", i32)]


class GemmTNJob(C.Structure):
    _fields_ = [("A", vp), ("B", vp), ("out", vp), ("R", i32), ("N", i32), ("K", i32), ("lda", i32), ("ldb", i32),
                ("ldo", i32), ("a_cols", i32), ("b_cols", i32)]


TN_MAX_JOBS = 16


class AttnArgs(C.Structure):
    _fields_ = [("Q", vp), ("K", vp), ("V", vp), ("O", vp), ("stat_m", vp), ("stat_l", vp),
                ("ldq", i32), ("ldk", i32), ("ldv", i32), ("ldo", i32),
                ("B", i32), ("H", i32), ("Nq", i32), ("Nk", i32), ("head_dim", i32), ("mask_kind", i32),
                ("scale", f32), ("causal", i32),
                ("kpad", vp), ("cs", vp), ("modq", vp), ("modk", vp), ("dense", vp),
                ("dO", vp), ("dQ", vp), ("dK", vp), ("dV", vp),
                ("lddo", i32), ("lddq", i32), ("lddk", i32), ("lddv", i32), ("force_tr", i32), ("kv_batch_rows", i32), ("zero_attn", i32)]


class AttnDecodeArgs(C.Structure):
    _fields_ = [("q", vp), ("k", vp), ("v", vp), ("o", vp), ("q_w", vp), ("q_b", vp), ("k_w", vp), ("k_b", vp), ("kpad", vp),
                ("ldq", i32), ("ldk", i32), ("ldv", i32), ("ldo", i32),
                ("B", i32), ("H", i32), ("Nk", i32), ("kv_batch_rows", i32), ("k_new_row", i32), ("is_f32", i32), ("zero_attn", i32), ("pad_", i32),
                ("scale", f32), ("eps", f32)]


class ModDesc(C.Structure):
    _fields_ = [("ids", vp), ("mask", vp), ("dam", vp), ("table", vp), ("pos", vp), ("mod_emb", vp), ("proj_bias", vp),
                ("L", i32), ("kind", i32), ("ids_are_i64", i32), ("mod_id", i32), ("max_len", i32), ("shifted", i32),
                ("mask_stride", i32), ("id_stride", i32), ("patch", i32), ("channels", i32), ("grid_w", i32),
                ("orig_dim", i32), ("head_index", i32), ("pad_", i32)]


class ShadowDesc(C.Structure):
    _fields_ = [("src", vp), ("dst", vp), ("ld_src", i32), ("ld_dst", i32), ("rows", i32), ("cols", i32),
                ("transpose", i32), ("tile_start", i32), ("col_scale", vp), ("dst_f32", i32), ("reserved", i32)]


FOLD_MAX_JOBS = 48


class FoldGradJob(C.Structure):
    _fields_ = [("dWp", vp), ("W", vp), ("gamma", vp), ("gW", vp), ("ggamma", vp), ("rows", i32), ("cols", i32), ("ld_dwp", i32), ("reserved", i32)]


class GemmF32Args(C.Structure):
    _fields_ = [("X", vp), ("W", vp), ("W2", vp), ("out", vp), ("out2", vp), ("res", vp), ("bias", vp), ("bias2", vp),
                ("sxm", i64), ("sxk", i64), ("swn", i64), ("swk", i64),
                ("M", i32), ("N", i32), ("K", i32), ("ldo", i32), ("ldo2", i32), ("ldr", i32), ("Hp", i32), ("epilogue", i32),
                ("accumulate", i32), ("max_N", i32), ("seg_rows", i32), ("n_groups", i32),
                ("groups", vp), ("tile_group", vp), ("seg_start", vp), ("seg_count", vp)]


class SpanMaskArgs(C.Structure):
    _fields_ = [("ids", vp), ("len", vp), ("unit", vp), ("noise", vp), ("keep_prob", vp), ("r_choice", vp), ("input_budget", vp), ("target_budget", vp),
                ("sentinel_ids", vp), ("emb", vp), ("emb_out", vp), ("src", vp), ("tensor", vp), ("input_mask", vp), ("target_mask", vp),
                ("decoder_attention_mask", vp), ("tries", vp),
                ("B", i32), ("ld_ids", i32), ("T", i32), ("ld_noise", i32), ("n_sentinels", i32), ("max_tokens", i32), ("vocab_offset", i32), ("pad_id", i32),
                ("emb_rows", i32), ("emb_dim", i32)]


class AdamWJob(C.Structure):
    _fields_ = [("p", vp), ("g", vp), ("m", vp), ("v", vp), ("dst_plain", vp), ("dst_t", vp),
                ("rows", i32), ("cols", i32), ("ld_plain", i32), ("ld_t", i32), ("tile_start", i32), ("pad_", i32)]


class SelectDesc(C.Structure):
    _fields_ = [("mods", ModDesc * FM_MAX_MODS),
                ("n_mods", i32), ("batch", i32), ("dim", i32), ("n_keep", i32), ("n_reg", i32), ("total_len", i32),
                ("is_decoder", i32), ("raw", i32),
                ("reg_tokens", vp), ("mask_token", vp),
                ("tokens", vp), ("emb", vp), ("x0", vp), ("out_mask", vp), ("out_mod", vp), ("slot_mod", vp),
                ("slot_src", vp), ("slot_pos", vp), ("target_ids", vp), ("out_cs", vp), ("out_mod_pre", vp),
                ("out_mod_index", vp), ("patch_rows", vp), ("seqemb_rows", vp), ("patch_ld", i32), ("seqemb_ld", i32),
                ("rows_f32", i32), ("pad2_", i32)]


class EmbedBwdMod(C.Structure):
    _fields_ = [("d_table", vp), ("d_pos", vp), ("d_mod_emb", vp), ("d_proj_bias", vp),
                ("kind", i32), ("has_padding_idx", i32), ("padding_idx", i32), ("pad_", i32)]


class EmbedBwdDesc(C.Structure):
    _fields_ = [("mods", EmbedBwdMod * FM_MAX_MODS), ("dx", vp), ("slot_mod", vp), ("slot_src", vp), ("slot_pos", vp),
                ("d_mask_token", vp), ("d_reg_tokens", vp),
                ("n_mods", i32), ("batch", i32), ("dim", i32), ("Nt", i32), ("lddx", i32), ("is_decoder", i32)]


class EmaJob(C.Structure):
    _fields_ = [("ema", vp), ("model", vp), ("n", i64), ("first_chunk", i64)]


class PilCropJob(C.Structure):
    _fields_ = [("src_off", i64), ("mid_off", i64), ("out_slot", i64), ("blk_rows", i64), ("blk_cols", i64), ("H", i32), ("W", i32), ("top", i32), ("left", i32),
                ("h", i32), ("w", i32), ("flip", i32), ("tab_w", i32), ("tab_h", i32), ("taps_w", i32), ("taps_h", i32), ("pad_", i32)]


def _sig(name, *argtypes):
    fn = getattr(lib, name)
    fn.argtypes = list(argtypes)
    fn.restype = C.c_int
    return fn


P = C.POINTER
gemm_nt = _sig("fm_gemm_nt", P(GemmNTArgs), vp)
gemm_tn = _sig("fm_gemm_tn", P(GemmTNArgs), vp)
gemm_tn_multi = _sig("fm_gemm_tn_multi", P(GemmTNJob), C.c_int, vp)
layernorm_fwd = _sig("fm_layernorm_fwd", vp, i32, vp, vp, vp, i32, i32, vp, vp, vp, i32, i32, f32, vp)
layernorm_fwd_res = _sig("fm_layernorm_fwd_res", vp, i32, vp, i32, vp, i32, vp, vp, vp, i32, i32, vp, vp, vp, i32, i32, f32, vp)
layernorm_bwd = _sig("fm_layernorm_bwd", vp, i32, vp, vp, i32, vp, vp, vp, vp, vp, i32, vp, i32, vp, vp, i32, i32, vp)
layernorm_bwd_h = _sig("fm_layernorm_bwd_h", vp, i32, vp, i32, vp, i32, vp, vp, vp, vp, vp, i32, vp, i32, vp, i32, i32, vp)
attn_fwd = _sig("fm_attn_fwd", P(AttnArgs), vp)
attn_bwd = _sig("fm_attn_bwd", P(AttnArgs), vp)
attn_decode = _sig("fm_attn_decode", P(AttnDecodeArgs), vp)
ATTN_DECODE_MAX_NK = 8192
select_embed = _sig("fm_select_embed", P(SelectDesc), vp)
embed_bwd = _sig("fm_embed_bwd", P(EmbedBwdDesc), vp)
dense_decoder_mask = _sig("fm_dense_decoder_mask", vp, vp, vp, i32, i32, i32, i32, i32, vp)
# ... 168 lines not shown
```

ml-4m_amd/fourm/hip/engine.py:

```python
import math
import os
import random
import weakref
from typing import Dict, List, Optional

import torch
import torch.nn as nn

from . import _lib as L
from . import ops

_WEIGHT_EPOCH = 0
FUSE_ACT_BWD = os.environ.get("FOURM_FUSE_ACT_BWD", "0") == "1"
HEADS_DENSE = os.environ.get("FOURM_HEADS_DENSE", "1") == "1"
HEADS_DENSE_MAX = int(os.environ.get("FOURM_HEADS_DENSE_MAX", "8"))
DEFER_RESIDUAL = os.environ.get("FOURM_DEFER_RESIDUAL", "1") == "1"
HOIST_CTX = os.environ.get("FOURM_HOIST_CTX", "1") == "1"
LN_BWD_FROM_H = os.environ.get("FOURM_LN_BWD_FROM_H", "1") == "1"
DP_RESERVE_ALWAYS = os.environ.get("FOURM_DP_RESERVE_ALWAYS", "0") == "1"


def bump_weight_epoch():
    global _WEIGHT_EPOCH
    _WEIGHT_EPOCH += 1


def ru(x, m):
    return (x + m - 1) // m * m


def is_lora(lin) -> bool:
    return hasattr(lin, "lora_down")


def check_lora_targets(model):
    from fourm.models.lora_utils import MAX_LORA_WIDTH, LoRAWrapper
    ok = set()
    for blk in model.encoder:
        ok |= {id(blk.attn.qkv), id(blk.attn.proj)}
    for blk in getattr(model, "decoder", ()):
        ok |= {id(blk.self_attn.qkv), id(blk.self_attn.proj), id(blk.cross_attn.q), id(blk.cross_attn.kv), id(blk.cross_attn.proj)}
    for name, mod in model.named_modules():
        if not isinstance(mod, LoRAWrapper):
            continue
        if id(mod) not in ok:
            raise NotImplementedError(f"LoRA wrapper at '{name}': the HIP engine adapts the attention Linears of the encoder / decoder blocks only "
                                      "(the MLP's fc1 / fc3 run as one launch whose SwiGLU epilogue consumes the pre-activation; embeddings and "
                                      "heads have no low-rank path)")
        width = mod.lora_down.weight.shape[0]
        if width > MAX_LORA_WIDTH:
            raise NotImplementedError(f"LoRA wrapper at '{name}': rank x packed Linears = {width} exceeds {MAX_LORA_WIDTH}")


class Shadow:
    __slots__ = ("buf", "params", "jobs", "stamp")

    def __init__(self, buf, params, jobs):
        self.buf, self.params, self.jobs, self.stamp = buf, params, jobs, None


class Workspace:

    def __init__(self, device, per_stream: bool = False):
        self.device = device
        self.per_stream = per_stream
        self.bufs: Dict[tuple, torch.Tensor] = {}

    def get(self, name, shape, dtype):
        key = (name, tuple(shape), dtype, torch.cuda.current_stream(self.device).cuda_stream) if self.per_stream else (name, tuple(shape), dtype)
        t = self.bufs.get(key)
        if t is None:
            t = self.bufs[key] = torch.zeros(shape, dtype=dtype, device=self.device)
        return t

    def nbytes(self):
        return sum(t.numel() * t.element_size() for t in self.bufs.values())


def fill_mod_desc(md, d, emb, is_dec: bool, mod_id: int, head_index: int = 0, raw: int = 0, name: str = "modality"):
    kind = emb.kind
    t = d["tensor"]
    B = t.shape[0]
    mask = d["target_mask" if is_dec else "input_mask"]
    mask = mask.reshape(B, -1)
    if mask.dtype != torch.bool:
        mask = mask.bool()
    mask = mask.contiguous()
    keep = [mask]
    md.mask, md.mask_stride = mask.data_ptr(), mask.shape[1]
    md.kind, md.mod_id, md.head_index = kind, mod_id, head_index
    md.pos = emb.pos_emb.data_ptr()
    md.mod_emb = emb.mod_emb.data_ptr()
    md.shifted = 1 if (is_dec and kind == L.KIND_SEQ and raw != 2) else 0
    md.max_len = getattr(emb, "max_length", 0) or 0
    if kind in (L.KIND_TOK, L.KIND_SEQ):
        ids = t.reshape(B, -1)
        if ids.dtype not in (torch.int32, torch.int64):
            ids = ids.long()
        ids = ids.contiguous()
        keep.append(ids)
        md.ids, md.ids_are_i64, md.id_stride = ids.data_ptr(), 1 if ids.dtype == torch.int64 else 0, ids.shape[1]
# ... 131 lines not shown
        claim("dec_emb", m.decoder_embeddings)
        claim("dec_emb", [m.mask_token])
        claim("ctx", m.decoder_proj_context)
        claim("ctx", m.encoder_norm)
        for i, blk in enumerate(m.encoder):
            claim(f"enc{i}", blk)
        claim("enc_emb", m.encoder_embeddings)
        if m.register_tokens is not None:
            claim("enc_emb", [m.register_tokens])
        stages = {}
        for n, p in self._named:
            o, k = self._slices[id(p)]
            stage = owner.get(id(p), "enc_emb") if k >= 65536 else "tail"
            stages.setdefault(stage, []).append((o, ru(k, 16)))
        return stages

    def _stage(self, name):
        if self.reducer is not None:
            self.reducer.stage_done(name)

    def grad_view(self, p):
        o, k = self._slices[id(p)]
        return self.flat_grads[o:o + k].view(p.shape)

    def grads_were_cleared(self) -> bool:
        live = getattr(self, "_attached", None)
        if not live:
            return True
        for p in live[:4] + live[-4:]:
            if p.grad is None or p.grad.data_ptr() != self.grad_view(p).data_ptr():
                return True
        return False

    def untouched_params(self):
        c = self._ctx
        if c is None or self.reducer is not None:
            return []
        m, touched, cand = self.model, set(), []
        for names, embs in ((c["enc"]["names"], m.encoder_embeddings), (c["dec"]["names"], m.decoder_embeddings)):
            for n, e in embs.items():
                if n in names:
                    touched.update(id(p) for p in e.parameters())
                else:
                    cand.extend(e.parameters())
        return [p for p in cand if id(p) not in touched]

    def attach_grads(self, zero: bool, untouched=()):
        if zero:
            with ops._prof("fills"):
                self.flat_grads.zero_()
            self._window_touched = set()
        skip = {id(p) for p in untouched} - getattr(self, "_window_touched", set())
        self._attached = []
        for n, p in self._named:
            if not p.requires_grad:
                continue
            if id(p) in skip:
                p.grad = None
                continue
            self._window_touched.add(id(p))
            p.grad = self.grad_view(p)
            self._attached.append(p)

    def _stamp(self, params):
        return tuple((p._version, _WEIGHT_EPOCH, p.data_ptr()) for p in params)

    def _get_shadow(self, key, make) -> torch.Tensor:
        s = self.shadows.get(key)
        if s is None:
            s = self.shadows[key] = make()
            for p in s.params:
                regs = getattr(p, "_fourm_shadows", None)
                if regs is None:
                    regs = p._fourm_shadows = []
                regs.append((weakref.ref(self), key))
        if s.stamp != self._stamp(s.params):
            self._refresh_shadows()
        return s.buf

    def _refresh_shadows(self):
        stale = [s for s in self.shadows.values() if s.stamp != self._stamp(s.params)]
        jobs = []
        for s in stale:
            jobs += [(j[0].detach().reshape(j[0].shape[0], -1), j[1], j[2], j[3].detach() if len(j) > 3 and j[3] is not None else None) for j in s.jobs]
        sig = tuple((a.data_ptr(), b.data_ptr(), tr, sc.data_ptr() if sc is not None else 0) for (a, b, tr, sc) in jobs)
        if self._shadow_table is None or self._shadow_table[0] != sig:
            table, tiles = ops.shadow_jobs_table(jobs, self.device)
            self._shadow_table = (sig, table, len(jobs), tiles)
        _, table, n, tiles = self._shadow_table
        ops.shadow_refresh(table, n, tiles)
        for s in stale:
            s.stamp = self._stamp(s.params)

    def mark_shadows_fresh(self, keys, written):
        for key in keys:
            s = self.shadows.get(key)
            if s is not None and all(len(j) == 3 and (id(j[0]), j[1].data_ptr()) in written for j in s.jobs):
                s.stamp = self._stamp(s.params)

    def w(self, p, pad_rows=False):
        if self.fp32:
            return p.detach().reshape(p.shape[0], -1)
        def make():
            out_f, in_f = p.shape[0], p[0].numel()
            buf = torch.zeros(ru(out_f, 64) if pad_rows else out_f, ru(in_f, 64), dtype=torch.bfloat16, device=p.device)
            return Shadow(buf, (p,), [(p, buf, False)])
        s = self._get_shadow(("w", id(p)), make)
        assert not pad_rows or s.shape[0] >= ru(p.shape[0], 64), "w(): the cached image was created without pad_rows"
        return s

    def wt(self, p, pad_rows=False):
        if self.fp32:
            return p.detach().reshape(p.shape[0], -1).t()
        def make():
            out_f, in_f = p.shape[0], p[0].numel()
            buf = torch.zeros(ru(in_f, 64) if pad_rows else in_f, ru(out_f, 64), dtype=torch.bfloat16, device=p.device)
            return Shadow(buf, (p,), [(p, buf, True)])
        s = self._get_shadow(("wt", id(p)), make)
        assert not pad_rows or s.shape[0] >= ru(p[0].numel(), 64), "wt(): the cached image was created without pad_rows"
        return s

    def w_fold(self, lin, norm):
        p, g = lin.weight, norm.weight
        def make():
            out_f, in_f = p.shape
            buf = torch.zeros(out_f, in_f if self.fp32 else ru(in_f, 64), dtype=self.adt, device=p.device)
            return Shadow(buf, (p, g), [(p, buf, False, g)])
        return self._get_shadow(("wfold", id(p)), make)

    def wt_fold_stack(self):
        m, D = self.model, self.D
        def make():
            Ld = len(m.decoder)
            buf = torch.zeros(D, Ld * 2 * D, dtype=self.adt, device=self.device)
            ps, jobs = [], []
            for i, blk in enumerate(m.decoder):
                p, g = blk.cross_attn.kv.weight, blk.context_norm.weight
                ps += [p, g]
                jobs.append((p, buf[:, i * 2 * D:(i + 1) * 2 * D], True, g))
            return Shadow(buf, tuple(ps), jobs)
        return self._get_shadow(("wtfold", 0), make)

    @property
    def hoist_ctx(self):
        h = getattr(self, "_hoist_ctx", None)
        if h is None:
            dec = getattr(self.model, "decoder", ())
            h = HOIST_CTX and len(dec) > 0 and all(
                not isinstance(b.context_norm.bias, nn.Parameter) and b.cross_attn.kv.bias is None and not is_lora(b.cross_attn.kv)
                for b in dec)
            self._hoist_ctx = h
        return h

    def w13t(self, mlp):
        def make():
            buf = torch.zeros(self.D, 2 * self.Hp, dtype=torch.bfloat16, device=self.device)
            p1, p3 = mlp.fc1.weight, mlp.fc3.weight
            return Shadow(buf, (p1, p3), [(p1, buf[:, :self.Hp], True), (p3, buf[:, self.Hp:], True)])
        return self._get_shadow(("w13t", id(mlp)), make)

    def _mod_desc(self, md: L.ModDesc, name, d, emb, is_dec, head_index=0, raw=0):
        return fill_mod_desc(md, d, emb, is_dec, int(self.model.modality_info[name]["id"]), head_index, raw, name)

    def select(self, mod_dict, n_keep: int, is_dec: bool, order: List[str], prefix: str, want_x0=True, heads=None, raw=0):
        m = self.model
        embs = m.decoder_embeddings if is_dec else m.encoder_embeddings
        names = [n for n in order if n in embs]
# ... 683 lines not shown
```

ml-4m_amd/fourm/hip/ops.py:

```python
import contextlib
import ctypes as C
import threading
from typing import Optional

import torch

from . import _lib as L

_PROFILER = None


def set_profiler(p):
    global _PROFILER
    _PROFILER = p


class _Null:
    def __enter__(self):
        return self

    def __exit__(self, *a):
        return False


# ... 391 lines not shown


def tap_add(g, dtap, g_bf=None, row_scale=None, rows_per_sample=0, R=None):
    R = g.shape[0] if R is None else R
    L.check(L.tap_add(_p(g), _ld(g), _p(g_bf), _ld(g_bf) if g_bf is not None else 0, _p(dtap), _ld(dtap), _p(row_scale), rows_per_sample, R, g.shape[1],
                      _stream()))
    return g


def feat_distance(pred, tgt, B, T, mode, loss, dpred):
    L.check(L.feat_distance(_p(pred), _ld(pred), _p(tgt), _ld(tgt), B, T, pred.shape[1], mode, _p(loss), _p(dpred), _ld(dpred), _stream()))
    return loss


def _is_f32(t):
    if t.dtype not in (torch.float32, torch.bfloat16):
        raise TypeError(f"feature rows are bf16 or f32, got {t.dtype}")
    return 1 if t.dtype == torch.float32 else 0


def lpips_stem(img, mul, add, w, bias, out, B, H, W):
    esz = out.element_size()
    with _prof("lpips_stem", 2.0 * B * H * W * 64 * 27, B * H * W * (12.0 + 64 * esz), tag=f"B{B} {H}x{W}"):
        L.check(L.lpips_stem(_p(img), _p(mul), _p(add), _p(w), _p(bias), _p(out), _ld(out), _is_f32(out), B, H, W, _stream()))
    return out


def lpips_stem_bwd(d, w, mul, row_scale, dimg, B, H, W):
    with _prof("lpips_stem_bwd", 2.0 * B * H * W * 64 * 27, B * H * W * (12.0 + 64 * d.element_size()), tag=f"B{B} {H}x{W}"):
        L.check(L.lpips_stem_bwd(_p(d), _ld(d), _is_f32(d), _p(w), _p(mul), _p(row_scale), _p(dimg), B, H, W, _stream()))
    return dimg


def maxpool2x2_nhwc(x, y, B, H, W, C):
    with _prof("maxpool2x2_nhwc", 0.0, 1.25 * B * H * W * C * x.element_size(), tag=f"B{B} {H}x{W} C{C}"):
        L.check(L.maxpool2x2_nhwc(_p(x), _ld(x), _p(y), _ld(y), _is_f32(x), B, H, W, C, _stream()))
    return y


def lpips_distance_scratch(B, P):
    return B * ((P + L.LPIPS_CHUNK - 1) // L.LPIPS_CHUNK)


def lpips_distance(pred, tgt, w, B, P, loss, dpred, scratch):
    C_ = pred.shape[1]
    assert scratch.dtype == torch.float32 and scratch.numel() >= lpips_distance_scratch(B, P) and _is_f32(pred) == _is_f32(tgt)
    with _prof("lpips_distance", 0.0, B * P * C_ * (2.0 * pred.element_size() + (4.0 if dpred is not None else 0.0)), tag=f"B{B} P{P} C{C_}"):
        L.check(L.lpips_distance(_p(pred), _ld(pred), _p(tgt), _ld(tgt), _is_f32(pred), _p(w), B, P, C_, _p(loss), _p(dpred),
                                 _ld(dpred) if dpred is not None else 0, _p(scratch), _stream()))
    return loss


def lpips_tap_bwd(act, d, B, H, W, din=None, dtap=None, dpool=None):
    C_ = act.shape[1]
    f = _is_f32(act)
    assert _is_f32(d) == f and (din is None or _is_f32(din) == f) and (dpool is None or _is_f32(dpool) == f) and (dtap is None or dtap.dtype == torch.float32)
    n_in = (din is not None) + (dpool is not None) * 0.25
    with _prof("lpips_tap_bwd", 0.0, B * H * W * C_ * ((2.0 + n_in) * act.element_size() + (4.0 if dtap is not None else 0.0)), tag=f"B{B} {H}x{W} C{C_}"):
        L.check(L.lpips_tap_bwd(_p(act), _ld(act), _p(din), _ld(din) if din is not None else 0, _p(dtap), _ld(dtap) if dtap is not None else 0,
                                _p(dpool), _ld(dpool) if dpool is not None else 0, _p(d), _ld(d), f, B, H, W, C_, _stream()))
    return d


def cast_pad(src, dst):
    s2 = src.reshape(src.shape[0], -1)
    L.check(L.cast_pad(_p(s2), s2.stride(0), _p(dst), _ld(dst), s2.shape[0], s2.shape[1], _stream()))
    return dst


def transpose_cast_pad(src, dst):
    s2 = src.reshape(src.shape[0], -1)
    L.check(L.transpose_cast_pad(_p(s2), s2.stride(0), _p(dst), _ld(dst), dst.shape[1], s2.shape[0], s2.shape[1], _stream()))
    return dst


def shadow_jobs_table(jobs, device):
    arr = (L.ShadowDesc * len(jobs))()
    tiles = 0
    for i, job in enumerate(jobs):
        src, dst, tr = job[:3]
        scale = job[3] if len(job) > 3 else None
        rows, cols = src.shape
        need = (cols, rows) if tr else (rows, cols)
        assert src.dtype == torch.float32 and dst.dtype in (torch.bfloat16, torch.float32) and src.stride(1) == 1 and dst.stride(1) == 1
        assert dst.shape[0] >= need[0] and dst.shape[1] >= need[1], (tuple(dst.shape), need)
        d = arr[i]
        d.src, d.dst, d.ld_src, d.ld_dst = src.data_ptr(), dst.data_ptr(), src.stride(0), dst.stride(0)
        d.rows, d.cols, d.transpose, d.tile_start = rows, cols, 1 if tr else 0, tiles
        d.dst_f32 = 1 if dst.dtype == torch.float32 else 0
        if scale is not None:
            assert scale.dtype == torch.float32 and scale.numel() == cols and scale.is_contiguous()
            d.col_scale = scale.data_ptr()
        tiles += ((rows + 63) // 64) * ((cols + 63) // 64)
    raw = torch.frombuffer(bytearray(bytes(arr)), dtype=torch.uint8).to(device)
    return raw, tiles


@_timed("fold_colscale_grad")
def fold_colscale_grad(jobs):
    for lo in range(0, len(jobs), L.FOLD_MAX_JOBS):
        part = jobs[lo:lo + L.FOLD_MAX_JOBS]
        arr = (L.FoldGradJob * len(part))()
        for j, (dwp, w, gamma, gw, gg) in zip(arr, part):
            rows, cols = w.shape[0], w[0].numel()
            assert w.is_contiguous() and (gw is None or gw.is_contiguous()) and dwp.stride(1) == 1
            j.dWp, j.W, j.gamma, j.gW, j.ggamma = _p(dwp), _p(w), _p(gamma), _p(gw), _p(gg)
            j.rows, j.cols, j.ld_dwp = rows, cols, dwp.stride(0)
        L.check(L.fold_colscale_grad(arr, len(part), _stream()))


@_timed("shadow_refresh")
def shadow_refresh(table, n_jobs, tiles):
    L.check(L.shadow_refresh(_p(table), n_jobs, tiles, _stream()))


@_timed("colsum")
def colsum(dy, db, N, R=None):
    if dy.dtype == torch.float32:
        return L.check(L.colsum_f32(_p(dy), _ld(dy), _p(db), dy.shape[0] if R is None else R, N, _stream()))
    L.check(L.colsum(_p(dy), _ld(dy), _p(db), dy.shape[0] if R is None else R, N, _stream()))


@_timed("casts")
def f32_to_bf16(src, dst):
    if dst.dtype == torch.float32:
        return dst.copy_(src)
    L.check(L.f32_to_bf16(_p(src), _p(dst), src.numel(), _stream()))
    return dst


@_timed("casts")
def bf16_to_f32_scaled(src, dst, scale=1.0):
    L.check(L.bf16_to_f32_scaled(_p(src), _p(dst), src.numel(), float(scale), _stream()))
    return dst


@_timed("drop_path")
def scale_rows_bf16(x, scale, rows_per_sample, R, N=None):
    L.check(L.scale_rows_bf16(_p(x), _ld(x), _p(scale), rows_per_sample, R, x.shape[1] if N is None else N, _stream()))
    return x


@_timed("casts")
def add_bf16_to_f32(x, delta, out, R=None):
    R = x.shape[0] if R is None else R
    assert x.is_contiguous() and delta.is_contiguous() and out.is_contiguous() and x.shape[1] == delta.shape[1] == out.shape[1]
    L.check(L.add_bf16_f32(_p(x), _p(delta), _p(out), R * x.shape[1], _stream()))
    return out


@_timed("adamw")
def adamw(p, g, m, v, n, lr, beta1, beta2, eps, wd, step, grad_mult=None, hyper=None, sumsq=None):
    L.check(L.adamw(_p(p), _p(g), _p(m), _p(v), n, lr, beta1, beta2, eps, wd, step, _p(grad_mult), _p(hyper), _p(sumsq), _stream()))


ADAMW_CHUNK = 8192


def adamw_jobs_table(jobs, device):
    arr = (L.AdamWJob * len(jobs))()
    tiles = 0
    for i, j in enumerate(jobs):
        p = j["p"]
        rows, cols = p.shape[0], p[0].numel()
        d = arr[i]
        for k in ("p", "g", "m", "v"):
            t = j[k]
            assert t.dtype == torch.float32 and t.is_contiguous() and t.numel() == rows * cols, (k, t.dtype, tuple(t.shape))
            setattr(d, k, t.data_ptr())
        pl, tr = j.get("plain"), j.get("t")
        if pl is not None:
            assert pl.dtype == torch.bfloat16 and pl.stride(1) == 1 and pl.shape[0] >= rows and pl.shape[1] >= cols
# ... 287 lines not shown
```

Measured before the change: 1.151 million tokens/s.

## Add pipelined shadow refresh, single-pass row segmentation, parallel loss finalize, line embed backward

Several independent kernel changes are added, each behind a lab flag that is on by default. Shadow weight refresh can now read from an already-fresh bf16 plain shadow instead of the fp32 master, and a new refresh kernel prefetches the next tile while writing the current one. Row segmentation becomes a single one-block kernel using wave ballots instead of three launches. Loss finalize runs as a parallel reduction, and embedding backward uses a new line-based kernel with per-wave run accumulators. Together these aim to cut memory traffic and launch count in small auxiliary kernels, at the cost of more code paths and a new dependency on shadow freshness ordering.

```diff
diff --git a/include/fourm_hip.h b/include/fourm_hip.h
--- a/include/fourm_hip.h
+++ b/include/fourm_hip.h
@@ -203,7 +203,7 @@
     const void* src; void* dst;
     int32_t ld_src, ld_dst, rows, cols, transpose, tile_start;
     const void* col_scale;
-    int32_t dst_f32, reserved;
+    int32_t dst_f32, src_bf16;
 } fm_shadow_desc;
 int fm_shadow_refresh(const fm_shadow_desc* descs, int n_descs, int total_tiles, void* stream);
 #define FM_FOLD_MAX_JOBS 48
diff --git a/ml-4m_amd/csrc/elementwise.hip b/ml-4m_amd/csrc/elementwise.hip
--- a/ml-4m_amd/csrc/elementwise.hip
+++ b/ml-4m_amd/csrc/elementwise.hip
@@ -1,5 +1,7 @@
 #include "common.h"
 #include "fourm_hip.h"
+
+int fm_lab_get(int key);
 
 namespace {
 
@@ -185,7 +187,11 @@
             const int gr = tr0 + p + 16 * i, gc = tc0 + q;
 #pragma unroll
             for (int e = 0; e < 4; ++e) v[i][e] = 0.f;
-            if (gr < d.rows) {
+            if (gr < d.rows && d.src_bf16) {
+                const bf16_t* sb = (const bf16_t*)d.src + (size_t)gr * d.ld_src + gc;
+#pragma unroll
+                for (int e = 0; e < 4; ++e) if (gc + e < d.cols) v[i][e] = bf2f(sb[e]);
+            } else if (gr < d.rows) {
                 const float* sp = src + (size_t)gr * d.ld_src + gc;
                 if (vec_src && gc + 3 < d.cols) {
                     const float4 f = *(const float4*)sp;
@@ -255,6 +261,140 @@
 #pragma unroll
                 for (int e = 0; e < 4; ++e) if (gr + e < d.rows) dp[e] = f2bf(tile[q + e][c]);
         }
+    }
+}
+
+__global__ __launch_bounds__(256) void shadow_refresh_lines_kernel(const fm_shadow_desc* __restrict__ descs, int n, int total_tiles) {
+    __shared__ float tile[64][65];
+    const int t_first = blockIdx.x * SHADOW_TILES_PER_BLOCK, t_end = min(total_tiles, t_first + SHADOW_TILES_PER_BLOCK);
+    int lo = 0, hi = n - 1;
+    while (lo < hi) {
+        const int mid = (lo + hi + 1) >> 1;
+        if (descs[mid].tile_start <= t_first) lo = mid; else hi = mid - 1;
+    }
+    fm_shadow_desc d = descs[lo];
+    int next_start = lo + 1 < n ? descs[lo + 1].tile_start : 0x7fffffff;
+    const int q = (threadIdx.x & 15) * 4, p = threadIdx.x >> 4;
+    auto load = [&](const fm_shadow_desc& j, int tt, uint4 (&raw)[4]) {
+        const int t = tt - j.tile_start, tiles_c = (j.cols + 63) / 64;
+        const int tr0 = (t / tiles_c) * 64, tc0 = (t % tiles_c) * 64, gc = tc0 + q;
+        const bool vec = (j.ld_src % 4 == 0) && ((((uintptr_t)j.src) & (j.src_bf16 ? 7 : 15)) == 0) && gc + 3 < j.cols;
+#pragma unroll
+        for (int i = 0; i < 4; ++i) {
+            const int gr = tr0 + p + 16 * i;
+            raw[i] = make_uint4(0u, 0u, 0u, 0u);
+            if (gr >= j.rows) continue;
+            if (j.src_bf16) {
+                const bf16_t* sb = (const bf16_t*)j.src + (size_t)gr * j.ld_src + gc;
+                if (vec) {
+                    const uint2 u = *(const uint2*)sb;
+                    raw[i].x = u.x; raw[i].y = u.y;
+                } else {
+                    uint32_t h[4] = {0u, 0u, 0u, 0u};
+#pragma unroll
+                    for (int e = 0; e < 4; ++e) if (gc + e < j.cols) h[e] = sb[e];
+                    raw[i].x = h[0] | (h[1] << 16); raw[i].y = h[2] | (h[3] << 16);
+                }
+            } else {
+                const float* sp = (const float*)j.src + (size_t)gr * j.ld_src + gc;
+                if (vec) raw[i] = *(const uint4*)sp;
+                else {
+                    uint32_t h[4] = {0u, 0u, 0u, 0u};
+#pragma unroll
+                    for (int e = 0; e < 4; ++e) if (gc + e < j.cols) h[e] = __float_as_uint(sp[e]);
+                    raw[i] = make_uint4(h[0], h[1], h[2], h[3]);
+                }
+            }
+        }
+    };
+    auto write = [&](const fm_shadow_desc& j, int tt, const uint4 (&raw)[4]) {
+        const int t = tt - j.tile_start, tiles_c = (j.cols + 63) / 64;
+        const int tr0 = (t / tiles_c) * 64, tc0 = (t % tiles_c) * 64;
+        bf16_t* dst = (bf16_t*)j.dst;
+        float v[4][4];
+#pragma unroll
+        for (int i = 0; i < 4; ++i) {
+            if (j.src_bf16) {
+                v[i][0] = bf2f((bf16_t)(raw[i].x & 0xffff)); v[i][1] = bf2f((bf16_t)(raw[i].x >> 16));
+                v[i][2] = bf2f((bf16_t)(raw[i].y & 0xffff)); v[i][3] = bf2f((bf16_t)(raw[i].y >> 16));
+            } else {
+                v[i][0] = __uint_as_float(raw[i].x); v[i][1] = __uint_as_float(raw[i].y);
+                v[i][2] = __uint_as_float(raw[i].z); v[i][3] = __uint_as_float(raw[i].w);
+            }
+        }
+        if (j.col_scale) {
+            const float* cs = (const float*)j.col_scale;
+#pragma unroll
+            for (int e = 0; e < 4; ++e) {
+                const float sc = tc0 + q + e < j.cols ? cs[tc0 + q + e] : 0.f;
+#pragma unroll
+                for (int i = 0; i < 4; ++i) v[i][e] *= sc;
+            }
+        }
+        if (j.dst_f32) {
+            float* df = (float*)j.dst;
+#pragma unroll
+            for (int i = 0; i < 4; ++i) {
+                const int gr = tr0 + p + 16 * i, gc = tc0 + q;
+                if (gr >= j.rows) continue;
+#pragma unroll
+                for (int e = 0; e < 4; ++e)
+                    if (gc + e < j.cols) df[j.transpose ? (size_t)(gc + e) * j.ld_dst + gr : (size_t)gr * j.ld_dst + gc + e] = v[i][e];
+            }
+            return;
+        }
+        if (!j.transpose) {
+            const bool vec_dst = ((((uintptr_t)dst) & 7) == 0) && (j.ld_dst % 4 == 0);
+#pragma unroll
+            for (int i = 0; i < 4; ++i) {
+                const int gr = tr0 + p + 16 * i, gc = tc0 + q;
+                if (gr >= j.rows) continue;
+                bf16_t* dp = dst + (size_t)gr * j.ld_dst + gc;
+                if (vec_dst && gc + 3 < j.cols) *(uint2*)dp = make_uint2(pack2bf(v[i][0], v[i][1]), pack2bf(v[i][2], v[i][3]));
+                else
+#pragma unroll
+                    for (int e = 0; e < 4; ++e) if (gc + e < j.cols) dp[e] = f2bf(v[i][e]);
+            }
+            return;
+        }
+        __syncthreads();
+#pragma unroll
+        for (int i = 0; i < 4; ++i)
+#pragma unroll
+            for (int e = 0; e < 4; ++e) tile[p + 16 * i][q + e] = v[i][e];
+        __syncthreads();
+        const bool vec_dst = ((((uintptr_t)dst) & 15) == 0) && (j.ld_dst % 8 == 0);
+#pragma unroll
+        for (int h = 0; h < 2; ++h) {
+            const int idx = threadIdx.x + 256 * h;
+            const int c = idx >> 3, r0 = (idx & 7) * 8;
+            const int gc = tc0 + c, gr = tr0 + r0;
+            if (gc >= j.cols) continue;
+            bf16_t* dp = dst + (size_t)gc * j.ld_dst + gr;
+            if (vec_dst && gr + 7 < j.rows)
+                *(uint4*)dp = make_uint4(pack2bf(tile[r0][c], tile[r0 + 1][c]), pack2bf(tile[r0 + 2][c], tile[r0 + 3][c]),
+                                         pack2bf(tile[r0 + 4][c], tile[r0 + 5][c]), pack2bf(tile[r0 + 6][c], tile[r0 + 7][c]));
+            else
+#pragma unroll
+                for (int e = 0; e < 8; ++e) if (gr + e < j.rows) dp[e] = f2bf(tile[r0 + e][c]);
+        }
+    };
+    uint4 cur[4], nxt[4];
+    load(d, t_first, cur);
+    for (int tt = t_first; tt < t_end; ++tt) {
+        fm_shadow_desc dn = d;
+        if (tt + 1 < t_end) {
+            if (tt + 1 >= next_start) {
+                ++lo;
+                dn = descs[lo];
+                next_start = lo + 1 < n ? descs[lo + 1].tile_start : 0x7fffffff;
+            }
+            load(dn, tt + 1, nxt);
+        }
+        write(d, tt, cur);
+        d = dn;
+#pragma unroll
+        for (int i = 0; i < 4; ++i) cur[i] = nxt[i];
     }
 }
 
@@ -537,8 +677,12 @@
 
 extern "C" int fm_shadow_refresh(const fm_shadow_desc* descs, int n_descs, int total_tiles, void* stream) {
     FM_CHECK_ARG(descs && n_descs > 0 && total_tiles > 0, "fm_shadow_refresh: bad argument");
-    hipLaunchKernelGGL(shadow_refresh_kernel, dim3((total_tiles + SHADOW_TILES_PER_BLOCK - 1) / SHADOW_TILES_PER_BLOCK), dim3(256), 0,
-                       (hipStream_t)stream, descs, n_descs, total_tiles);
+    if (fm_lab_get(14))
+        hipLaunchKernelGGL(shadow_refresh_lines_kernel, dim3((total_tiles + SHADOW_TILES_PER_BLOCK - 1) / SHADOW_TILES_PER_BLOCK), dim3(256), 0,
+                           (hipStream_t)stream, descs, n_descs, total_tiles);
+    else
+        hipLaunchKernelGGL(shadow_refresh_kernel, dim3((total_tiles + SHADOW_TILES_PER_BLOCK - 1) / SHADOW_TILES_PER_BLOCK), dim3(256), 0,
+                           (hipStream_t)stream, descs, n_descs, total_tiles);
     FM_CHECK_LAUNCH("fm_shadow_refresh");
     return 0;
 }
diff --git a/ml-4m_amd/csrc/gemm.hip b/ml-4m_amd/csrc/gemm.hip
--- a/ml-4m_amd/csrc/gemm.hip
+++ b/ml-4m_amd/csrc/gemm.hip
@@ -1003,7 +1003,10 @@
                  [] { const char* e = getenv("FOURM_NT4"); return e ? atoi(e) : 1; }(),
                  [] { const char* e = getenv("FOURM_TN4"); return e ? atoi(e) : 0; }(), 0, 0, 0,
                  [] { const char* e = getenv("FOURM_NT_SMALL"); return e ? atoi(e) : 1; }(),
-                 [] { const char* e = getenv("FOURM_CONV_K32"); return e ? atoi(e) : 1; }()};
+                 [] { const char* e = getenv("FOURM_CONV_K32"); return e ? atoi(e) : 1; }(),
+                 [] { const char* e = getenv("FOURM_EMBED_BWD_LINES"); return e ? atoi(e) : 1; }(), 0,
+                 [] { const char* e = getenv("FOURM_LOSS_GLUE"); return e ? atoi(e) : 1; }(),
+                 [] { const char* e = getenv("FOURM_SHADOW_LINES"); return e ? atoi(e) : 1; }()};
 int g_nt_swiglu = 12;
 int g_nt_auto[2] = {11, 10};
 
@@ -1277,6 +1280,7 @@
 }
 extern "C" int fm_get_gemm_nt_config(void) { return g_nt_config; }
 extern "C" void fm_lab_set(int key, int value) { if (key >= 0 && key < 16) g_lab[key] = value; }
+int fm_lab_get(int key) { return key >= 0 && key < 16 ? g_lab[key] : 0; }
 extern "C" void fm_set_reserved_cus(int n) { g_reserved_cus = n < 0 ? 0 : n; }
 extern "C" int fm_get_reserved_cus(void) { return g_reserved_cus; }
 static int g_tn_config = [] { const char* e = getenv("FOURM_TN_CONFIG"); return e ? atoi(e) : 1; }();
diff --git a/ml-4m_amd/csrc/loss.hip b/ml-4m_amd/csrc/loss.hip
--- a/ml-4m_amd/csrc/loss.hip
+++ b/ml-4m_amd/csrc/loss.hip
@@ -1,5 +1,7 @@
 #include "common.h"
 #include "fourm_hip.h"
+
+int fm_lab_get(int key);
 
 namespace {
 
@@ -46,6 +48,84 @@
             row_to_padded[r] = dst;
         }
         run += tot;
+    }
+}
+
+constexpr int SEG_CACHE = 48 * 1024;
+
+__global__ __launch_bounds__(1024) void segment_rows_once_kernel(const int32_t* __restrict__ head_of_row, int R, int n_heads,
+                                                                 int32_t* __restrict__ seg_start, int32_t* __restrict__ seg_count,
+                                                                 int32_t* __restrict__ perm, int32_t* __restrict__ row_to_padded,
+                                                                 int32_t* __restrict__ tile_group, int Rp) {
+    __shared__ int8_t hc[SEG_CACHE];
+    __shared__ int wcnt[16][FM_MAX_MODS];
+    __shared__ int sstart[FM_MAX_MODS + 1], scount[FM_MAX_MODS];
+    const int tid = threadIdx.x, lane = tid & 63, wave = tid >> 6;
+    const bool cached = R <= SEG_CACHE;
+    const int rw = ((R + 15) / 16 + 63) / 64 * 64;
+    const int r_lo = min(R, wave * rw), r_hi = min(R, r_lo + rw);
+    auto valid = [&](int h) { return h >= 0 && h < n_heads; };
+    int cnt = 0;
+    for (int base = r_lo; base < r_hi; base += 16 * 64) {
+        int h[16];
+#pragma unroll
+        for (int u = 0; u < 16; ++u) { const int r = base + 64 * u + lane; h[u] = r < r_hi ? head_of_row[r] : -1; }
+#pragma unroll
+        for (int u = 0; u < 16; ++u) {
+            const int r = base + 64 * u + lane;
+            if (!valid(h[u])) h[u] = -1;
+            if (cached && r < r_hi) hc[r] = (int8_t)h[u];
+            for (int g = 0; g < n_heads; ++g) {
+                const unsigned long long bal = __ballot(h[u] == g);
+                if (lane == g) cnt += __popcll(bal);
+            }
+        }
+    }
+    if (lane < n_heads) wcnt[wave][lane] = cnt;
+    __syncthreads();
+    if (tid < n_heads) {
+        int c = 0;
+        for (int w = 0; w < 16; ++w) c += wcnt[w][tid];
+        scount[tid] = c;
+    }
+    __syncthreads();
+    if (tid == 0) {
+        int s = 0;
+        for (int g = 0; g < n_heads; ++g) { sstart[g] = s; s += (scount[g] + SEG_ALIGN - 1) / SEG_ALIGN * SEG_ALIGN; }
+        sstart[n_heads] = s;
+    }
+    __syncthreads();
+    if (tid < n_heads) { seg_start[tid] = sstart[tid]; seg_count[tid] = scount[tid]; }
+    for (int g = 0; g < n_heads; ++g) {
+        const int start = sstart[g], end = sstart[g + 1];
+        for (int t = start / SEG_ALIGN + tid; t < end / SEG_ALIGN; t += 1024) tile_group[t] = g;
+        for (int r = start + scount[g] + tid; r < end; r += 1024) perm[r] = -1;
+    }
+    for (int t = sstart[n_heads] / SEG_ALIGN + tid; t < Rp / SEG_ALIGN; t += 1024) tile_group[t] = -1;
+    for (int r = sstart[n_heads] + tid; r < Rp; r += 1024) perm[r] = -1;
+    int next = 0;
+    if (lane < n_heads) {
+        next = sstart[lane];
+        for (int w = 0; w < wave; ++w) next += wcnt[w][lane];
+    }
+    for (int base = r_lo; base < r_hi; base += 64) {
+        const int r = base + lane;
+        int h = -1;
+        if (r < r_hi) {
+            h = cached ? (int)hc[r] : head_of_row[r];
+            if (!valid(h)) h = -1;
+        }
+        int dst = -1;
+        for (int g = 0; g < n_heads; ++g) {
+            const unsigned long long bal = __ballot(h == g);
+            const int first = __builtin_amdgcn_readlane(next, g);
+            if (h == g) dst = first + __popcll(bal & ((1ull << lane) - 1ull));
+            if (lane == g) next += __popcll(bal);
+        }
+        if (r < r_hi) {
+            row_to_padded[r] = dst;
+            if (dst >= 0) perm[dst] = r;
+        }
     }
 }
 
@@ -181,6 +261,41 @@
     }
 }
 
+__global__ __launch_bounds__(1024) void loss_finalize_par_kernel(const float* __restrict__ row_loss, const int32_t* __restrict__ seg_start,
+                                                                 const int32_t* __restrict__ seg_count, const int32_t* __restrict__ vocab,
+                                                                 int n_heads, int loss_type, float* __restrict__ head_loss, float* __restrict__ total) {
+    __shared__ float red[FM_MAX_MODS][4];
+    const int t = threadIdx.x & 255, lane = threadIdx.x & 63, wave = (threadIdx.x >> 6) & 3, q = threadIdx.x >> 8;
+    for (int g = q; g < n_heads; g += 4) {
+        const int s0 = seg_start[g], n = seg_count[g];
+        float s = 0.f;
+#pragma unroll 8
+        for (int i = t; i < n; i += 256) s += row_loss[s0 + i];
+        s = wave_sum(s);
+        if (lane == 0) red[g][wave] = s;
+    }
+    __syncthreads();
+    if (threadIdx.x == 0) {
+        float tot = 0.f, wsum = 0.f;
+        for (int g = 0; g < n_heads; ++g) {
+            const int n = seg_count[g];
+            const float hl = n > 0 ? ((red[g][0] + red[g][1]) + (red[g][2] + red[g][3])) / (float)n : 0.f;
+            head_loss[g] = hl;
+            if (loss_type == FM_LOSS_MOD) { tot += hl; wsum += 1.f; }
+            else { const float w = (float)n * (float)vocab[g]; tot += hl * w; wsum += w; }
+        }
+        total[0] = tot / wsum;
+    }
+}
+
+void launch_loss_finalize(const float* row_loss, const int32_t* seg_start, const int32_t* seg_count, const int32_t* vocab, int n_heads, int loss_type,
+                          float* head_loss, float* total, hipStream_t stream) {
+    if (fm_lab_get(13))
+        hipLaunchKernelGGL(loss_finalize_par_kernel, dim3(1), dim3(1024), 0, stream, row_loss, seg_start, seg_count, vocab, n_heads, loss_type, head_loss, total);
+    else
+        hipLaunchKernelGGL(loss_finalize_kernel, dim3(1), dim3(256), 0, stream, row_loss, seg_start, seg_count, vocab, n_heads, loss_type, head_loss, total);
+}
+
 __global__ __launch_bounds__(256) void ce_f32_kernel(float* logits, int ld, const int* perm, const int* tile_group, const long long* target_ids,
                                                      const int* vocab, const int* seg_count, const float* grad_scale, int loss_type, int n_heads,
                                                      float* row_loss, float* row_lse, int write_grad, int seg_rows) {
@@ -250,6 +365,12 @@
     FM_CHECK_ARG(n_heads > 0 && n_heads <= FM_MAX_MODS && R > 0, "fm_segment_rows: bad shape");
     FM_CHECK_ARG(Rp % SEG_ALIGN == 0 && Rp >= (R + SEG_ALIGN - 1) / SEG_ALIGN * SEG_ALIGN + (n_heads - 1) * SEG_ALIGN,
                  "fm_segment_rows: padded capacity Rp=%d too small for R=%d rows in %d segments", Rp, R, n_heads);
+    if (fm_lab_get(13)) {
+        hipLaunchKernelGGL(segment_rows_once_kernel, dim3(1), dim3(1024), 0, (hipStream_t)stream, head_of_row, R, n_heads, seg_start, seg_count, perm,
+                           row_to_padded, tile_group, Rp);
+        FM_CHECK_LAUNCH("fm_segment_rows");
+        return 0;
+    }
     hipLaunchKernelGGL(fill_i32_kernel, dim3((R + 255) / 256), dim3(256), 0, (hipStream_t)stream, row_to_padded, -1, R);
     hipLaunchKernelGGL(segment_rows_kernel, dim3(n_heads), dim3(1024), 0, (hipStream_t)stream, head_of_row, R, n_heads, seg_start,
                        seg_count, perm, row_to_padded, tile_group, Rp);
@@ -278,8 +399,8 @@
     if (!write_grad) {
         hipLaunchKernelGGL(ce_fwd_kernel, dim3(Rp), dim3(256), 0, (hipStream_t)stream, (const bf16_t*)logits, ldl, perm, tile_group,
                            (const long long*)target_ids, vocab, (float*)row_loss, (float*)row_lse);
-        hipLaunchKernelGGL(loss_finalize_kernel, dim3(1), dim3(256), 0, (hipStream_t)stream, (const float*)row_loss, seg_start, seg_count,
-                           vocab, n_heads, loss_type, (float*)head_loss, (float*)total_loss);
+        launch_loss_finalize((const float*)row_loss, seg_start, seg_count, vocab, n_heads, loss_type, (float*)head_loss, (float*)total_loss,
+                             (hipStream_t)stream);
     } else {
         hipLaunchKernelGGL(ce_bwd_kernel, dim3(Rp), dim3(256), 0, (hipStream_t)stream, (bf16_t*)logits, ldl, perm, tile_group,
                            (const long long*)target_ids, vocab, seg_count, (const float*)grad_scale, loss_type, n_heads, (const float*)row_lse);
@@ -300,8 +421,8 @@
                        (const long long*)target_ids, vocab, seg_count, (const float*)grad_scale, loss_type, n_heads, (float*)row_loss,
                        (float*)row_lse, write_grad, SEG_ALIGN);
     if (!write_grad)
-        hipLaunchKernelGGL(loss_finalize_kernel, dim3(1), dim3(256), 0, (hipStream_t)stream, (const float*)row_loss, seg_start, seg_count,
-                           vocab, n_heads, loss_type, (float*)head_loss, (float*)total_loss);
+        launch_loss_finalize((const float*)row_loss, seg_start, seg_count, vocab, n_heads, loss_type, (float*)head_loss, (float*)total_loss,
+                             (hipStream_t)stream);
     FM_CHECK_LAUNCH("fm_cross_entropy_f32");
     return 0;
 }
diff --git a/ml-4m_amd/csrc/select_embed.hip b/ml-4m_amd/csrc/select_embed.hip
--- a/ml-4m_amd/csrc/select_embed.hip
+++ b/ml-4m_amd/csrc/select_embed.hip
@@ -1,5 +1,7 @@
 #include "common.h"
 #include "fourm_hip.h"
+
+int fm_lab_get(int key);
 
 namespace {
 
@@ -329,6 +331,143 @@
         for (int c = threadIdx.x; c < D; c += 256) unsafeAtomicAdd((float*)d.d_mask_token + c, acc[(size_t)d.n_mods * D + c]);
 }
 
+template <int K, int NF, bool SCATTER>
+__global__ __launch_bounds__(256) void embed_bwd_lines_kernel(fm_embed_bwd_desc d, int rpw) {
+    extern __shared__ __attribute__((aligned(16))) char smem[];
+    const int D = d.dim, rows = d.n_mods + 1;
+    float* acc = (float*)smem;
+    float* runs = acc + (size_t)rows * D;
+    __shared__ int used[FM_MAX_MODS + 1];
+    __shared__ int run_tag[4][2];
+    const int b = blockIdx.x, lane = threadIdx.x & 63, wave = threadIdx.x >> 6;
+    for (int i = threadIdx.x; i < rows * D; i += 256) acc[i] = 0.f;
+    if (threadIdx.x <= FM_MAX_MODS) used[threadIdx.x] = 0;
+    __syncthreads();
+    const int parts = 4 * gridDim.y, part = wave + 4 * blockIdx.y;
+    const int per = (d.Nt + parts - 1) / parts, s_lo = part * per, s_hi = min(d.Nt, s_lo + per);
+    float racc[K];
+    int cur = -1, tag0 = -1, tag1 = -1;
+    bool cur_mask = false;
+    auto flush = [&]() {
+        if (cur < 0) return;
+        const int tag = cur | (cur_mask ? 256 : 0);
+        int r = -1;
+        if (tag0 == tag) r = 0;
+        else if (tag1 == tag) r = 1;
+        if (r >= 0) {
+            float* slot = runs + (size_t)(wave * rpw + r) * D;
+#pragma unroll
+            for (int k = 0; k < K; ++k) { const int c = lane + 64 * k; if (c < D) slot[c] += racc[k]; }
+        } else if (tag0 < 0 && rpw > 0) {
+            tag0 = tag;
+            float* slot = runs + (size_t)(wave * rpw) * D;
+#pragma unroll
+            for (int k = 0; k < K; ++k) { const int c = lane + 64 * k; if (c < D) slot[c] = racc[k]; }
+        } else if (tag1 < 0 && rpw > 1) {
+            tag1 = tag;
+            float* slot = runs + (size_t)(wave * rpw + 1) * D;
+#pragma unroll
+            for (int k = 0; k < K; ++k) { const int c = lane + 64 * k; if (c < D) slot[c] = racc[k]; }
+        } else {
+#pragma unroll
+            for (int k = 0; k < K; ++k) {
+                const int c = lane + 64 * k;
+                if (c >= D) continue;
+                atomicAdd(acc + (size_t)cur * D + c, racc[k]);
+                if (cur_mask) atomicAdd(acc + (size_t)d.n_mods * D + c, racc[k]);
+            }
+        }
+    };
+    const int32_t* smod = (const int32_t*)d.slot_mod;
+    const int32_t* ssrc = (const int32_t*)d.slot_src;
+    const int32_t* spos = (const int32_t*)d.slot_pos;
+    for (int s0 = s_lo; s0 < s_hi; s0 += NF) {
+        float v[NF][K];
+        int mm[NF], src[NF], pos[NF];
+#pragma unroll
+        for (int f = 0; f < NF; ++f) {
+            mm[f] = -1; src[f] = 0; pos[f] = 0;
+            if (s0 + f >= s_hi) continue;
+            const size_t row = (size_t)b * d.Nt + s0 + f;
+            mm[f] = smod[row];
+            if (SCATTER) { src[f] = ssrc[row]; pos[f] = spos[row]; }
+            const float* g = (const float*)d.dx + row * d.lddx + lane;
+            if (D == 64 * K) {
+#pragma unroll
+                for (int k = 0; k < K; ++k) v[f][k] = g[64 * k];
+            } else {
+#pragma unroll
+                for (int k = 0; k < K; ++k) v[f][k] = lane + 64 * k < D ? g[64 * k] : 0.f;
+            }
+        }
+#pragma unroll
+        for (int f = 0; f < NF; ++f) {
+            const int m = __builtin_amdgcn_readfirstlane(mm[f]);
+            if (m == -1) continue;
+            if (m == -2) {
+                if (SCATTER && d.d_reg_tokens) {
+                    float* rrow = (float*)d.d_reg_tokens + (size_t)(s0 + f) * D;
+#pragma unroll
+                    for (int k = 0; k < K; ++k) { const int c = lane + 64 * k; if (c < D) unsafeAtomicAdd(rrow + c, v[f][k]); }
+                }
+                continue;
+            }
+            const fm_embed_bwd_mod& md = d.mods[m];
+            const bool to_mask_token = d.is_decoder && md.kind == FM_KIND_TOK;
+            if (m != cur) {
+                flush();
+                cur = m; cur_mask = to_mask_token;
+#pragma unroll
+                for (int k = 0; k < K; ++k) racc[k] = 0.f;
+                if (lane == 0) { used[m] = 1; if (to_mask_token) used[d.n_mods] = 1; }
+            }
+            float* trow = nullptr;
+            float* prow = nullptr;
+            if (SCATTER) {
+                const int sr = __builtin_amdgcn_readfirstlane(src[f]), ps = __builtin_amdgcn_readfirstlane(pos[f]);
+                if (to_mask_token) {}
+                else if ((md.kind == FM_KIND_TOK || md.kind == FM_KIND_SEQ) && md.d_table && !(md.has_padding_idx && sr == md.padding_idx))
+                    trow = (float*)md.d_table + (size_t)sr * D;
+                else if (md.kind == FM_KIND_SEQ_EMB && md.d_proj_bias) trow = (float*)md.d_proj_bias;
+                if (md.d_pos) prow = (float*)md.d_pos + (size_t)ps * D;
+            }
+#pragma unroll
+            for (int k = 0; k < K; ++k) {
+                const int c = lane + 64 * k;
+                if (c >= D) continue;
+                racc[k] += v[f][k];
+                if (SCATTER && trow) unsafeAtomicAdd(trow + c, v[f][k]);
+                if (SCATTER && prow) unsafeAtomicAdd(prow + c, v[f][k]);
+            }
+        }
+    }
+    flush();
+    if (lane == 0) { run_tag[wave][0] = tag0; run_tag[wave][1] = tag1; }
+    __syncthreads();
+    for (int m = 0; m <= d.n_mods; ++m) {
+        float* dst = m < d.n_mods ? (float*)d.mods[m].d_mod_emb : (float*)d.d_mask_token;
+        if (!used[m] || !dst) continue;
+        for (int c = threadIdx.x; c < D; c += 256) {
+            float s = acc[(size_t)m * D + c];
+#pragma unroll
+            for (int w = 0; w < 4; ++w)
+#pragma unroll
+                for (int r = 0; r < 2; ++r) {
+                    const int tag = run_tag[w][r];
+                    if (tag >= 0 && (m < d.n_mods ? (tag & 255) == m : (tag >> 8) != 0)) s += runs[(size_t)(w * rpw + r) * D + c];
+                }
+            unsafeAtomicAdd(dst + c, s);
+        }
+    }
+}
+
+template <int K, int NF, bool SCATTER>
+void launch_embed_bwd_lines(const fm_embed_bwd_desc* d, int rpw, size_t lds, dim3 grid, hipStream_t stream) {
+    static bool once = (hipFuncSetAttribute((const void*)embed_bwd_lines_kernel<K, NF, SCATTER>, hipFuncAttributeMaxDynamicSharedMemorySize, 150 * 1024) == hipSuccess);
+    (void)once;
+    hipLaunchKernelGGL((embed_bwd_lines_kernel<K, NF, SCATTER>), grid, dim3(256), lds, stream, *d, rpw);
+}
+
 __global__ void dense_decoder_mask_kernel(const int32_t* cs, const int16_t* mod, uint8_t* out, int B, int M, int causal, int use_cs, int use_sep) {
     const size_t i = (size_t)blockIdx.x * 256 + threadIdx.x;
     if (i >= (size_t)B * M * M) return;
@@ -385,6 +524,28 @@
     static bool once = (hipFuncSetAttribute((const void*)embed_bwd_kernel, hipFuncAttributeMaxDynamicSharedMemorySize, 150 * 1024) == hipSuccess);
     (void)once;
     const int slices = d->batch >= 2048 ? 1 : d->batch >= 1024 ? 2 : 4;
+    if (fm_lab_get(11)) {
+        bool scatter = d->d_reg_tokens != nullptr;
+        for (int m = 0; m < d->n_mods; ++m) scatter = scatter || d->mods[m].d_table || d->mods[m].d_pos || d->mods[m].d_proj_bias;
+        const size_t slot = (size_t)4 * d->dim * sizeof(float);
+        const int rpw = lds + 2 * slot <= 150 * 1024 ? 2 : lds + slot <= 150 * 1024 ? 1 : 0;
+        const size_t lds2 = lds + rpw * slot;
+        const dim3 grid(d->batch, slices);
+        const int groups = (d->dim + 63) / 64;
+        hipStream_t s = (hipStream_t)stream;
+#define FM_EB_LAUNCH(K, NFS)                                                     \
+    do {                                                                         \
+        if (scatter) launch_embed_bwd_lines<K, 2, true>(d, rpw, lds2, grid, s);  \
+        else launch_embed_bwd_lines<K, NFS, false>(d, rpw, lds2, grid, s);       \
+    } while (0)
+        if (groups <= 4) FM_EB_LAUNCH(4, 4);
+        else if (groups <= 12) FM_EB_LAUNCH(12, 4);
+        else if (groups <= 16) FM_EB_LAUNCH(16, 2);
+        else FM_EB_LAUNCH(32, 2);
+#undef FM_EB_LAUNCH
+        FM_CHECK_LAUNCH("fm_embed_bwd");
+        return 0;
+    }
     hipLaunchKernelGGL(embed_bwd_kernel, dim3(d->batch, slices), dim3(256), lds, (hipStream_t)stream, *d);
     FM_CHECK_LAUNCH("fm_embed_bwd");
     return 0;
diff --git a/ml-4m_amd/fourm/hip/_lib.py b/ml-4m_amd/fourm/hip/_lib.py
--- a/ml-4m_amd/fourm/hip/_lib.py
+++ b/ml-4m_amd/fourm/hip/_lib.py
@@ -85,7 +85,7 @@
 
 class ShadowDesc(C.Structure):
     _fields_ = [("src", vp), ("dst", vp), ("ld_src", i32), ("ld_dst", i32), ("rows", i32), ("cols", i32),
-                ("transpose", i32), ("tile_start", i32), ("col_scale", vp), ("dst_f32", i32), ("reserved", i32)]
+                ("transpose", i32), ("tile_start", i32), ("col_scale", vp), ("dst_f32", i32), ("src_bf16", i32)]
 
 
 FOLD_MAX_JOBS = 48
diff --git a/ml-4m_amd/fourm/hip/engine.py b/ml-4m_amd/fourm/hip/engine.py
--- a/ml-4m_amd/fourm/hip/engine.py
+++ b/ml-4m_amd/fourm/hip/engine.py
@@ -17,6 +17,7 @@
 DEFER_RESIDUAL = os.environ.get("FOURM_DEFER_RESIDUAL", "1") == "1"
 HOIST_CTX = os.environ.get("FOURM_HOIST_CTX", "1") == "1"
 LN_BWD_FROM_H = os.environ.get("FOURM_LN_BWD_FROM_H", "1") == "1"
+SHADOW_FROM_PLAIN = os.environ.get("FOURM_SHADOW_FROM_PLAIN", "1") == "1"
 DP_RESERVE_ALWAYS = os.environ.get("FOURM_DP_RESERVE_ALWAYS", "0") == "1"
 
 
@@ -314,7 +315,13 @@
         stale = [s for s in self.shadows.values() if s.stamp != self._stamp(s.params)]
         jobs = []
         for s in stale:
-            jobs += [(j[0].detach().reshape(j[0].shape[0], -1), j[1], j[2], j[3].detach() if len(j) > 3 and j[3] is not None else None) for j in s.jobs]
+            for j in s.jobs:
+                src, scale = j[0].detach().reshape(j[0].shape[0], -1), j[3].detach() if len(j) > 3 and j[3] is not None else None
+                if SHADOW_FROM_PLAIN and scale is None and j[1].dtype == torch.bfloat16:
+                    pl = self.shadows.get(("w", id(j[0])))
+                    if pl is not None and pl is not s and pl.stamp == self._stamp(pl.params) and pl.buf.dtype == torch.bfloat16:
+                        src = pl.buf[:src.shape[0], :src.shape[1]]
+                jobs.append((src, j[1], j[2], scale))
         sig = tuple((a.data_ptr(), b.data_ptr(), tr, sc.data_ptr() if sc is not None else 0) for (a, b, tr, sc) in jobs)
         if self._shadow_table is None or self._shadow_table[0] != sig:
             table, tiles = ops.shadow_jobs_table(jobs, self.device)
diff --git a/ml-4m_amd/fourm/hip/ops.py b/ml-4m_amd/fourm/hip/ops.py
--- a/ml-4m_amd/fourm/hip/ops.py
+++ b/ml-4m_amd/fourm/hip/ops.py
@@ -497,12 +497,14 @@
         scale = job[3] if len(job) > 3 else None
         rows, cols = src.shape
         need = (cols, rows) if tr else (rows, cols)
-        assert src.dtype == torch.float32 and dst.dtype in (torch.bfloat16, torch.float32) and src.stride(1) == 1 and dst.stride(1) == 1
+        assert src.dtype in (torch.float32, torch.bfloat16) and dst.dtype in (torch.bfloat16, torch.float32) and src.stride(1) == 1 and dst.stride(1) == 1
+        assert src.dtype == torch.float32 or (dst.dtype == torch.bfloat16 and scale is None), "a bf16 source is copied as it stands"
         assert dst.shape[0] >= need[0] and dst.shape[1] >= need[1], (tuple(dst.shape), need)
         d = arr[i]
         d.src, d.dst, d.ld_src, d.ld_dst = src.data_ptr(), dst.data_ptr(), src.stride(0), dst.stride(0)
         d.rows, d.cols, d.transpose, d.tile_start = rows, cols, 1 if tr else 0, tiles
         d.dst_f32 = 1 if dst.dtype == torch.float32 else 0
+        d.src_bf16 = 1 if src.dtype == torch.bfloat16 else 0
         if scale is not None:
             assert scale.dtype == torch.float32 and scale.numel() == cols and scale.is_contiguous()
             d.col_scale = scale.data_ptr()
```

New measurement: 1.161 million tokens/s, median of 6. No clear change (+0.9%).
